# rainerzufalldererste/limg

Measured on AMD Instinct MI355X. Metric: encode Mpixels/s, 8K RGBA (limg_encode3d_test-equivalent: all 11 planes stored), higher is better.
Workload: dtype u8/i32 integer stage + f32 float stage (bit-exact vs the reference's strict SSE build)

## Files before the change

limg_amd/csrc/limg_hip_blocked.hip:

```cpp
#include "limg_hip_device.h"

namespace limg_hip
{
  namespace
  {
    __device__ __forceinline__ void scratch_fence()
    {
      __builtin_amdgcn_fence(__ATOMIC_RELEASE, "workgroup");
      __builtin_amdgcn_fence(__ATOMIC_ACQUIRE, "workgroup");
    }

    struct MState { float nA[4], nB[4], nC[4], invA, invB, invC; };

    template <int CH>
    __device__ __forceinline__ float dot_seq(const float *a, const float *b)
    {
      float sum = 0.0f;
#pragma unroll
      for (int i = 0; i < CH; i++) sum += a[i] * b[i];
      return sum;
    }

    template <int CH>
    __device__ __forceinline__ void m_init(const limg_hip_block_record &r, MState &s)
    {
      bool nzA = false, nzB = false, nzC = false;
#pragma unroll
      for (int i = 0; i < 4; i++) { s.nA[i] = 0.0f; s.nB[i] = 0.0f; s.nC[i] = 0.0f; }
#pragma unroll
      for (int i = 0; i < CH; i++)
      {
        s.nA[i] = (float)((int)r.dirA_max[i] - (int)r.dirA_min[i]);
        s.nB[i] = (float)((int)r.dirB_mag[i] - (int)r.dirB_offset[i]);
        s.nC[i] = (float)((int)r.dirC_mag[i] - (int)r.dirC_offset[i]);
        nzA |= s.nA[i] != 0; nzB |= s.nB[i] != 0; nzC |= s.nC[i] != 0;
      }
      s.invA = nzA ? 1.0f / dot_seq<CH>(s.nA, s.nA) : 0.0f;
      s.invB = nzB ? 1.0f / dot_seq<CH>(s.nB, s.nB) : 0.0f;
      s.invC = nzC ? 1.0f / dot_seq<CH>(s.nC, s.nC) : 0.0f;
    }

    template <int CH>
    __device__ __forceinline__ void m_factors(const float *color, const limg_hip_block_record &in, const MState &s, float f[3])
    {
      float t[4], est[4];
#pragma unroll
      for (int i = 0; i < CH; i++) t[i] = color[i] - (float)in.dirA_min[i];
      f[0] = dot_seq<CH>(t, s.nA) * s.invA;
#pragma unroll
      for (int i = 0; i < CH; i++) { est[i] = (float)in.dirA_min[i] + f[0] * s.nA[i]; t[i] = (color[i] - est[i]) - (float)in.dirB_offset[i]; }
      f[1] = dot_seq<CH>(t, s.nB) * s.invB;
#pragma unroll
      for (int i = 0; i < CH; i++) { est[i] = est[i] + f[1] * s.nB[i]; t[i] = (color[i] - est[i]) - (float)in.dirC_offset[i]; }
      f[2] = dot_seq<CH>(t, s.nC) * s.invC;
    }

    template <typename T>
    __device__ __forceinline__ float2_t splat2(T v) { return float2_t{ (float)v, (float)v }; }
    __device__ __forceinline__ float2_t pair2(float x, float y) { return float2_t{ x, y }; }

    template <int CH, typename TA, typename TB>
    __device__ __forceinline__ float2_t dot_seq2(const TA *a, const TB *b)
    {
      float2_t sum = { 0.0f, 0.0f };
#pragma unroll
      for (int i = 0; i < CH; i++) sum += a[i] * b[i];
      return sum;
    }

    template <int CH, typename TC, typename TR>
    __device__ __forceinline__ void m_factors2(const TC *color, const TR *mnA, const TR *ofB, const TR *ofC, const TR *nA, const TR *nB, const TR *nC, TR invA, TR invB, TR invC,
                                               float2_t f[3])
    {
      float2_t t[4], est[4];
#pragma unroll
      for (int i = 0; i < CH; i++) t[i] = color[i] - mnA[i];
      f[0] = dot_seq2<CH>(t, nA) * invA;
#pragma unroll
      for (int i = 0; i < CH; i++) { est[i] = mnA[i] + f[0] * nA[i]; t[i] = (color[i] - est[i]) - ofB[i]; }
      f[1] = dot_seq2<CH>(t, nB) * invB;
#pragma unroll
      for (int i = 0; i < CH; i++) { est[i] = est[i] + f[1] * nB[i]; t[i] = (color[i] - est[i]) - ofC[i]; }
      f[2] = dot_seq2<CH>(t, nC) * invC;
    }

    template <int CH>
    __device__ void m_matches_pair(const limg_hip_block_record &a, const limg_hip_block_record &b0, const limg_hip_block_record &b1, bool &r0, bool &r1)
    {
      MState sa;
      m_init<CH>(a, sa);
      float amnA[4], aofB[4], aofC[4];
      float2_t nA[4], nB[4], nC[4], mnA[4], ofB[4], ofC[4], avgB[4];
#pragma unroll
      for (int i = 0; i < CH; i++)
      {
        amnA[i] = (float)a.dirA_min[i]; aofB[i] = (float)a.dirB_offset[i]; aofC[i] = (float)a.dirC_offset[i];
        nA[i] = pair2((float)((int)b0.dirA_max[i] - (int)b0.dirA_min[i]), (float)((int)b1.dirA_max[i] - (int)b1.dirA_min[i]));
        nB[i] = pair2((float)((int)b0.dirB_mag[i] - (int)b0.dirB_offset[i]), (float)((int)b1.dirB_mag[i] - (int)b1.dirB_offset[i]));
        nC[i] = pair2((float)((int)b0.dirC_mag[i] - (int)b0.dirC_offset[i]), (float)((int)b1.dirC_mag[i] - (int)b1.dirC_offset[i]));
        mnA[i] = pair2((float)b0.dirA_min[i], (float)b1.dirA_min[i]);
        ofB[i] = pair2((float)b0.dirB_offset[i], (float)b1.dirB_offset[i]);
        ofC[i] = pair2((float)b0.dirC_offset[i], (float)b1.dirC_offset[i]);
        avgB[i] = pair2(b0.avg[i], b1.avg[i]);
      }
      float2_t invBA = 1.0f / dot_seq2<CH>(nA, nA), invBB = 1.0f / dot_seq2<CH>(nB, nB), invBC = 1.0f / dot_seq2<CH>(nC, nC);
      {
        bool zA0 = true, zA1 = true, zB0 = true, zB1 = true, zC0 = true, zC1 = true;
#pragma unroll
        for (int i = 0; i < CH; i++)
        {
          zA0 &= nA[i].x == 0.0f; zA1 &= nA[i].y == 0.0f; zB0 &= nB[i].x == 0.0f; zB1 &= nB[i].y == 0.0f; zC0 &= nC[i].x == 0.0f; zC1 &= nC[i].y == 0.0f;
        }
        invBA = pair2(zA0 ? 0.0f : invBA.x, zA1 ? 0.0f : invBA.y);
        invBB = pair2(zB0 ? 0.0f : invBB.x, zB1 ? 0.0f : invBB.y);
        invBC = pair2(zC0 ? 0.0f : invBC.x, zC1 ? 0.0f : invBC.y);
      }
      const float w[4] = { 2, 4, 3, 3 };
      float lenA[3] = { 3, 3, 3 };
      float2_t avgDiffSq = { 0, 0 }, lenB[3] = { { 3, 3 }, { 3, 3 }, { 3, 3 } };
#pragma unroll
      for (int i = 0; i < CH; i++)
      {
        const float2_t d = a.avg[i] - avgB[i];
        avgDiffSq += d * d * w[i];
        lenA[0] += (sa.nA[i] * sa.nA[i]) * w[i]; lenB[0] += (nA[i] * nA[i]) * w[i];
        lenA[1] += (sa.nB[i] * sa.nB[i]) * w[i]; lenB[1] += (nB[i] * nB[i]) * w[i];
        lenA[2] += (sa.nC[i] * sa.nC[i]) * w[i]; lenB[2] += (nC[i] * nC[i]) * w[i];
      }
      const float sumA = lenA[0] + lenA[1] + lenA[2];
      const float2_t sumB = lenB[0] + lenB[1] + lenB[2];
      const float2_t ratio = (sumA + 1) / (sumB + 1);
      const float maxAvg = (float)(16 * 3 * CH), maxRange = (float)(200 * 3 * CH);
      const bool q0 = avgDiffSq.x < maxAvg && sumA < maxRange && sumB.x < maxRange, q1 = avgDiffSq.y < maxAvg && sumA < maxRange && sumB.y < maxRange;
      const bool j0 = ratio.x > 1.375f || ratio.x < (1.f / 1.375f), j1 = ratio.y > 1.375f || ratio.y < (1.f / 1.375f);
      r0 = q0; r1 = q1;
      if ((q0 || j0) && (q1 || j1)) return;
      float invA[3];
      float2_t invB[3];
#pragma unroll
      for (int i = 0; i < 3; i++) { invA[i] = 1.0f / lenA[i]; invB[i] = 1.0f / lenB[i]; }
#pragma unroll
      for (int i = 1; i < 3; i++) { invA[i] *= 2.f; invB[i] *= 2.f; }
      float2_t fb[3];
      m_factors2<CH>(a.avg, mnA, ofB, ofC, nA, nB, nC, invBA, invBB, invBC, fb);
      const float2_t termB = __builtin_elementwise_abs(fb[0]) * invB[0] + __builtin_elementwise_abs(0.5f - fb[1]) * invB[1] + __builtin_elementwise_abs(0.5f - fb[2]) * invB[2];
      float2_t sum = { 0, 0 };
#pragma unroll 1
      for (int z = 0; z < 3; z++)
#pragma unroll 1
        for (int y = 0; y < 3; y++)
#pragma unroll
          for (int x = 0; x < 3; x++)
          {
            const float xf = x * 0.5f, yf = y * 0.5f, zf = z * 0.5f;
            float2_t color[4], fa[3];
#pragma unroll
            for (int i = 0; i < CH; i++) color[i] = nA[i] * xf + nB[i] * yf + nC[i] * zf;
            m_factors2<CH>(color, amnA, aofB, aofC, sa.nA, sa.nB, sa.nC, sa.invA, sa.invB, sa.invC, fa);
            sum += __builtin_elementwise_abs(fa[0]) * invA[0] + __builtin_elementwise_abs(0.5f - fa[1]) * invA[1] + __builtin_elementwise_abs(0.5f - fa[2]) * invA[2];
            sum += termB;
          }
      const float2_t avgF = sum * (1.f / 27);
      if (!q0 && !j0) r0 = avgF.x < 3.0f;
      if (!q1 && !j1) r1 = avgF.y < 3.0f;
    }

    template <int CH>
    __device__ __forceinline__ int m_early(const limg_hip_block_record &a, const MState &sa, const limg_hip_block_record &b)
    {
      MState sb;
      m_init<CH>(b, sb);
      const float w[4] = { 2, 4, 3, 3 };
      float avgDiffSq = 0, lenA[3] = { 3, 3, 3 }, lenB[3] = { 3, 3, 3 };
#pragma unroll
      for (int i = 0; i < CH; i++)
      {
        const float d = a.avg[i] - b.avg[i];
        avgDiffSq += d * d * w[i];
        lenA[0] += (sa.nA[i] * sa.nA[i]) * w[i]; lenB[0] += (sb.nA[i] * sb.nA[i]) * w[i];
        lenA[1] += (sa.nB[i] * sa.nB[i]) * w[i]; lenB[1] += (sb.nB[i] * sb.nB[i]) * w[i];
        lenA[2] += (sa.nC[i] * sa.nC[i]) * w[i]; lenB[2] += (sb.nC[i] * sb.nC[i]) * w[i];
      }
      const float sumA = lenA[0] + lenA[1] + lenA[2], sumB = lenB[0] + lenB[1] + lenB[2];
      const float ratio = (sumA + 1) / (sumB + 1);
      const float maxAvg = (float)(16 * 3 * CH), maxRange = (float)(200 * 3 * CH);
      if (avgDiffSq < maxAvg && sumA < maxRange && sumB < maxRange) return 1;
      if (ratio > 1.375f || ratio < (1.f / 1.375f)) return 2;
      return 0;
    }

    __device__ __forceinline__ void cell_to_block(const BlockedParams &p, uint32_t sx, uint32_t sy, int cell, bool &ok, size_t &idx)
    {
      const int dy = cell / kMatchSide - kMatchLo, dx = cell - (cell / kMatchSide) * kMatchSide - kMatchLo;
      const uint32_t cx = sx + (uint32_t)dx, cy = sy + (uint32_t)dy;
      ok = cell < kMatchCells && (dx | dy) != 0 && cx < p.blocksX && cy < p.blocksY;
      idx = ok ? (size_t)cy * p.blocksX + cx : 0;
    }

    template <int CH>
    __global__ __launch_bounds__(256) void k_blocked_bounds(const BlockedParams p)
    {
      const uint32_t i = blockIdx.x * 256 + threadIdx.x;
      if (i >= p.blocksX * p.blocksY) return;
      const limg_hip_block_record r = p.pass1[i];
      MState s;
      m_init<CH>(r, s);
      const float w[4] = { 2, 4, 3, 3 };
      float len[3] = { 3, 3, 3 }, qA = 0, qB = 0, qC = 0, qM = 0, qOB = 0, qOC = 0;
#pragma unroll
      for (int k = 0; k < CH; k++)
      {
        len[0] += (s.nA[k] * s.nA[k]) * w[k]; len[1] += (s.nB[k] * s.nB[k]) * w[k]; len[2] += (s.nC[k] * s.nC[k]) * w[k];
        qA += s.nA[k] * s.nA[k]; qB += s.nB[k] * s.nB[k]; qC += s.nC[k] * s.nC[k];
        const float m = (float)r.dirA_min[k], ob = (float)r.dirB_offset[k], oc = (float)r.dirC_offset[k];
        qM += m * m; qOB += ob * ob; qOC += oc * oc;
      }
      const float NA = sqrtf(qA), NB = sqrtf(qB), NC = sqrtf(qC), OB = sqrtf(qOB), OC = sqrtf(qOC);
      float alpha = 0.5f * 2.0f / len[1] + 0.5f * 2.0f / len[2], beta = 0;
      if (qA > 0) beta += 1.0f / (NA * len[0]);
      if (qB > 0) { alpha += (OB / NB) * 2.0f / len[1]; beta += 4.0f / (NB * len[1]); }
      if (qC > 0) { alpha += ((OB + OC) / NC) * 2.0f / len[2]; beta += 8.0f / (NC * len[2]); }
      reinterpret_cast<float4 *>(p.matchBound)[i] = make_float4(alpha, beta, sqrtf(qM), (NA + NB + NC) * 1.0001f);
    }

    template <int CH>
    __global__ __launch_bounds__(256, 3) void k_blocked_match(const BlockedParams p)
    {
      __shared__ unsigned short sList[4][kMatchWords * 64];
      __shared__ unsigned long long sWords[4][kMatchWords];
      const int wave = threadIdx.x >> 6;
      const uint32_t seed = p.seedBase + blockIdx.x * 4 + wave;
      const int lane = lane_id();
      if (seed >= p.seedBase + p.seedCount) return;
      const uint32_t sy = seed / p.blocksX, sx = seed - sy * p.blocksX;
      const limg_hip_block_record a = p.pass1[seed];
      MState sa;
      m_init<CH>(a, sa);
      float boundA = 0, boundB = 0, boundM = 0, boundAvg = 0, boundT0 = 0;
      if (p.matchBound)
      {
        const float4 ba = reinterpret_cast<const float4 *>(p.matchBound)[seed];
        float q = 0;
#pragma unroll
        for (int k = 0; k < CH; k++) q += a.avg[k] * a.avg[k];
        boundA = ba.x; boundB = ba.y; boundM = ba.z; boundAvg = sqrtf(q);
        const float w[4] = { 2, 4, 3, 3 }, zero[4] = { 0, 0, 0, 0 };
        float len[3] = { 3, 3, 3 }, f0[3];
#pragma unroll
        for (int k = 0; k < CH; k++) { len[0] += (sa.nA[k] * sa.nA[k]) * w[k]; len[1] += (sa.nB[k] * sa.nB[k]) * w[k]; len[2] += (sa.nC[k] * sa.nC[k]) * w[k]; }
        m_factors<CH>(zero, a, sa, f0);
        boundT0 = fabsf(f0[0]) * (1.0f / len[0]) + fabsf(0.5f - f0[1]) * ((1.0f / len[1]) * 2.f) + fabsf(0.5f - f0[2]) * ((1.0f / len[2]) * 2.f);
      }
      uint32_t count = 0;
      for (int c = 0; c < kMatchWords; c++)
      {
        const int cell = c * 64 + lane;
        bool ok;
        size_t idx;
        cell_to_block(p, sx, sy, cell, ok, idx);
        int e = 2;
        if (ok) e = m_early<CH>(a, sa, p.pass1[idx]);
        if (e == 0 && p.matchBound)
        {
          const float4 bb = reinterpret_cast<const float4 *>(p.matchBound)[idx];
          const float UA = boundA + boundB * (bb.w + boundM), U = UA + (bb.x + bb.y * (boundAvg + bb.z));
          if (U * 1.01f < 2.5f) e = 1;
          else if (boundT0 - 1.01f * (0.5f * boundB * bb.w) - 0.01f * UA > 3.01f) e = 2;
        }
        const unsigned long long yes = __builtin_amdgcn_ballot_w64(e == 1), open = __builtin_amdgcn_ballot_w64(e == 0);
        if (lane == 0) sWords[wave][c] = yes;
        if (e == 0) sList[wave][count + __builtin_amdgcn_mbcnt_hi((uint32_t)(open >> 32), __builtin_amdgcn_mbcnt_lo((uint32_t)open, 0u))] = (unsigned short)cell;
        count += (uint32_t)__builtin_popcountll(open);
      }
      wave_lds_fence();
      for (uint32_t k = 0; k < count; k += 128)
      {
        const uint32_t i0 = k + lane, i1 = k + 64 + lane;
        const bool v0 = i0 < count, v1 = i1 < count;
        const int cell0 = sList[wave][v0 ? i0 : 0], cell1 = sList[wave][v1 ? i1 : 0];
        bool ok0, ok1, r0 = false, r1 = false;
        size_t idx0, idx1;
        cell_to_block(p, sx, sy, cell0, ok0, idx0);
        cell_to_block(p, sx, sy, cell1, ok1, idx1);
        m_matches_pair<CH>(a, p.pass1[idx0], p.pass1[idx1], r0, r1);
        if (v0 && r0) atomicOr(&sWords[wave][cell0 >> 6], 1ull << (cell0 & 63));
        if (v1 && r1) atomicOr(&sWords[wave][cell1 >> 6], 1ull << (cell1 & 63));
      }
      wave_lds_fence();
      if (lane < kMatchWords) p.matchBits[(size_t)seed * kMatchWords + lane] = sWords[wave][lane];
      if (lane == 0)
      {
        auto bit = [&](int dx, int dy) -> uint32_t { const int cell = (dy + kMatchLo) * kMatchSide + dx + kMatchLo; return (uint32_t)(sWords[wave][cell >> 6] >> (cell & 63)) & 1u; };
        const uint32_t all8 = bit(1, 0) & bit(2, 0) & bit(0, 1) & bit(1, 1) & bit(2, 1) & bit(0, 2) & bit(1, 2) & bit(2, 2);
        p.matchFlags[seed] = (uint8_t)(all8 | ((bit(1, 0) | bit(0, 1)) << 1));
      }
    }

    struct Geo { uint32_t px0, py0, xpx, ypx, n; };

    __device__ __forceinline__ Geo region_geo(const BlockedParams &p, const RegionDesc &R)
    {
      Geo g;
      g.px0 = R.ox * kBlock; g.py0 = R.oy * kBlock;
      g.xpx = R.rx * kBlock; g.ypx = R.ry * kBlock;
      if (R.ox + R.rx == p.blocksX && (p.sizeX % kBlock)) g.xpx = g.xpx - kBlock + p.sizeX % kBlock;
      if (R.oy + R.ry == p.blocksY && (p.sizeY % kBlock)) g.ypx = g.ypx - kBlock + p.sizeY % kBlock;
      g.n = g.xpx * g.ypx;
      return g;
    }

    __device__ __forceinline__ float bcast(float v, int l) { return __int_as_float(__builtin_amdgcn_readlane(__float_as_int(v), l)); }

    __device__ __forceinline__ uint64_t wave_sum64(uint64_t v)
    {
      const uint32_t lo = (uint32_t)v, hi = (uint32_t)(v >> 32);
      return (uint64_t)wave_sum(lo & 0xFFFFu) + ((uint64_t)wave_sum(lo >> 16) << 16) + ((uint64_t)wave_sum(hi) << 32);
    }

    template <int CH>
    __global__ __launch_bounds__(64) void k_blocked_fit_search(const BlockedParams p)
    {
      __shared__ __attribute__((aligned(16))) float s_park[4][64 + 4];
      const uint32_t r = p.order ? p.order[blockIdx.x] : blockIdx.x;
      const int lane = lane_id();
      const RegionDesc R = p.regions[r];
      const Geo g = region_geo(p, R);
      const uint32_t n = g.n, cap = p.scratchCap;
      uint32_t *spx = p.scratchPx + R.scratch;
      uint8_t *sf = p.scratchFac + R.scratch;
      const unsigned short *tab = d_rsqrt_x86_tab;

      uint32_t s0 = 0, s1 = 0, s2 = 0, s3 = 0;
      for (uint32_t i = lane; i < n; i += 64)
      {
        const uint32_t row = i / g.xpx, col = i - row * g.xpx;
        const uint32_t px = p.in[(size_t)(g.py0 + row) * p.sizeX + g.px0 + col];
        spx[i] = px;
        s0 += px & 0xFF; s1 += (px >> 8) & 0xFF; s2 += (px >> 16) & 0xFF; s3 += px >> 24;
      }
      scratch_fence();

      limg_hip_block_record rec;
      memset(&rec, 0, sizeof(rec));
      if (R.keep)
      {
        rec = p.pass1[(size_t)R.oy * p.blocksX + R.ox];
      }
      else
      {
        s0 = wave_sum(s0); s1 = wave_sum(s1); s2 = wave_sum(s2); s3 = wave_sum(s3);
        const float inv_count = 1.0f / (float)n;
        V4 avg;
        avg.a = float2_t{ (float)(int)s0, (float)(int)s2 } * inv_count;
        avg.b = float2_t{ (float)(int)s1, CH == 4 ? (float)(int)s3 : 0.0f } * inv_count;
        const V4 zero4 = { float2_t{ 0.0f, 0.0f }, float2_t{ 0.0f, 0.0f } };
        V4 dirA = zero4, dirB = zero4, dirC = zero4;
        float mm[6] = { 0, 0, 0, 0, 0, 0 };
        bool zeroA = true, zeroB = true, zeroC = true;

        float walk = 0.0f;
        auto park_and_walk = [&](const V4 &u, uint32_t count ) {
          s_park[0][lane] = u.a.x; s_park[1][lane] = u.a.y; s_park[2][lane] = u.b.x; s_park[3][lane] = u.b.y;
          wave_lds_fence();
          if (lane < 4)
          {
            const float *src = s_park[lane];
            if (count == 64u)
            {
#pragma unroll
              for (int h = 0; h < 4; h++)
              {
                float4 v[4];
#pragma unroll
                for (int q = 0; q < 4; q++) v[q] = *reinterpret_cast<const float4 *>(src + 16 * h + 4 * q);
#pragma unroll
                for (int q = 0; q < 4; q++) { walk = walk + v[q].x; walk = walk + v[q].y; walk = walk + v[q].z; walk = walk + v[q].w; }
              }
            }
            else
              for (uint32_t i = 0; i < count; i++) walk = walk + src[i];
          }
          wave_lds_fence();
        };
        auto serial_sum = [&]() -> V4 {
          const float s = walk * inv_count;
          walk = 0.0f;
          V4 d;
          d.a = float2_t{ bcast(s, 0), bcast(s, 1) };
          d.b = float2_t{ bcast(s, 2), bcast(s, 3) };
          return d;
        };
        auto is_zero = [](const V4 &d) { return d.a.x == 0.0f && d.a.y == 0.0f && d.b.x == 0.0f && d.b.y == 0.0f; };

        for (uint32_t base = 0; base < n; base += 64)
        {
          const uint32_t i = base + lane;
          const bool active = i < n;
          const V4 pf = px_to_v4(active ? spx[i] : 0u);
          V4 d = pf - avg;
          mask_alpha<CH>(d);
          const V4 u = unit4<CH>(tab, d, active);
          park_and_walk(u, min(64u, n - base));
        }
        dirA = serial_sum();
        zeroA = is_zero(dirA);
        if (!zeroA)
        {
          const float invA = 1.0f / dp4<CH>(dirA, dirA);
          float mn = 0.0f, mx = 0.0f;
          for (uint32_t base = 0; base < n; base += 64)
          {
            const uint32_t i = base + lane;
            const bool active = i < n;
            const V4 pf = px_to_v4(active ? spx[i] : 0u);
            const float fA = dp4<CH>(pf - avg, dirA) * invA;
            if (active) { mn = vmin(mn, fA); mx = vmax(mx, fA); }
            V4 e = pf - (avg + dirA * fA);
            mask_alpha<CH>(e);
            const V4 u = unit4<CH>(tab, e, active);
            park_and_walk(u, min(64u, n - base));
          }
          wave_min_max(mn, mx);
          mm[0] = mn; mm[1] = mx;
          dirB = serial_sum();
          zeroB = is_zero(dirB);
          if (!zeroB)
          {
            const float invB = 1.0f / dp4<CH>(dirB, dirB);
            float mnB = FLT_MAX, mxB = -FLT_MAX, mnC = FLT_MAX, mxC = -FLT_MAX;
            if (CH == 4)
            {
              V4 est0 = zero4;
              for (uint32_t base = 0; base < n; base += 64)
              {
                const uint32_t i = base + lane;
                const bool active = i < n;
                const V4 pf = px_to_v4(active ? spx[i] : 0u);
                const float fA = dp4<CH>(pf - avg, dirA) * invA;
                const V4 est = avg + dirA * fA;
                const float fB = dp4<CH>(pf - est, dirB) * invB;
                if (active) { mnB = vmin(mnB, fB); mxB = vmax(mxB, fB); }
                const V4 est2 = est + dirB * fB;
                const V4 u = unit4<CH>(tab, pf - est2, active);
                park_and_walk(u, min(64u, n - base));
                if (base == 0) est0 = est2;
              }
              wave_min_max(mnB, mxB);
              est0.a = float2_t{ bcast(est0.a.x, 0), bcast(est0.a.y, 0) };
              est0.b = float2_t{ bcast(est0.b.x, 0), bcast(est0.b.y, 0) };
              dirC = serial_sum();
              zeroC = is_zero(dirC);
              if (!zeroC)
              {
                const float invC = 1.0f / dp4<CH>(dirC, dirC);
                for (uint32_t base = 0; base < n; base += 64)
                {
                  const uint32_t i = base + lane;
                  const bool active = i < n;
                  const V4 pf = px_to_v4(active ? spx[i] : 0u);
                  const float fC = dp4<CH>(pf - est0, dirC) * invC;
                  if (active) { mnC = vmin(mnC, fC); mxC = vmax(mxC, fC); }
                }
                wave_min_max(mnC, mxC);
              }
            }
            else
            {
              dirC.a.x = dirA.b.x * dirB.a.y - dirA.a.y * dirB.b.x;
              dirC.b.x = dirA.a.y * dirB.a.x - dirA.a.x * dirB.a.y;
              dirC.a.y = dirA.a.x * dirB.b.x - dirA.b.x * dirB.a.x;
              dirC.b.y = 0.0f;
              zeroC = dirC.a.x == 0.0f && dirC.b.x == 0.0f && dirC.a.y == 0.0f;
              const float invC = zeroC ? 0.0f : 1.0f / dp4<CH>(dirC, dirC);
              for (uint32_t base = 0; base < n; base += 64)
              {
                const uint32_t i = base + lane;
                const bool active = i < n;
                const V4 pf = px_to_v4(active ? spx[i] : 0u);
                const float fA = dp4<CH>(pf - avg, dirA) * invA;
                const V4 est = avg + dirA * fA;
                const float fB = dp4<CH>(pf - est, dirB) * invB;
                if (active) { mnB = vmin(mnB, fB); mxB = vmax(mxB, fB); }
                if (!zeroC)
                {
                  const V4 e = pf - (est + dirB * fB);
                  const float fC = dp4<CH>(e, dirC) * invC;
                  if (active) { mnC = vmin(mnC, fC); mxC = vmax(mxC, fC); }
                }
              }
              wave_min_max(mnB, mxB);
              if (!zeroC) wave_min_max(mnC, mxC);
            }
            mm[2] = mnB; mm[3] = mxB;
            if (!zeroC) { mm[4] = mnC; mm[5] = mxC; }
          }
        }
        const float av[4] = { avg.a.x, avg.b.x, avg.a.y, avg.b.y };
        const float dA[4] = { dirA.a.x, dirA.b.x, dirA.a.y, dirA.b.y }, dB[4] = { dirB.a.x, dirB.b.x, dirB.a.y, dirB.b.y }, dC[4] = { dirC.a.x, dirC.b.x, dirC.a.y, dirC.b.y };
        const bool deadA = zeroA, deadB = zeroA || zeroB, deadC = deadB || zeroC;
#pragma unroll
        for (int c = 0; c < 4; c++)
        {
          rec.avg[c] = (CH == 3 && c == 3) ? 0.0f : av[c];
          if (CH == 3 && c == 3) continue;
          rec.dirA_min[c] = (int16_t)cvt_rne(av[c] + (deadA ? 0.0f : mm[0] * dA[c]));
          rec.dirA_max[c] = (int16_t)cvt_rne(av[c] + (deadA ? 0.0f : mm[1] * dA[c]));
          rec.dirB_offset[c] = (int16_t)cvt_rne(deadB ? 0.0f : mm[2] * dB[c]);
          rec.dirB_mag[c] = (int16_t)cvt_rne(deadB ? 0.0f : mm[3] * dB[c]);
          rec.dirC_offset[c] = (int16_t)cvt_rne(deadC ? 0.0f : mm[4] * dC[c]);
          rec.dirC_mag[c] = (int16_t)cvt_rne(deadC ? 0.0f : mm[5] * dC[c]);
        }
      }

      const int16_t *lo3[3] = { rec.dirA_min, rec.dirB_offset, rec.dirC_offset }, *hi3[3] = { rec.dirA_max, rec.dirB_mag, rec.dirC_mag };
      V4 nrm[3], off[3];
      float invN[3];
      RecU ru;
#pragma unroll
      for (int f = 0; f < 3; f++)
      {
        float nv[4], ov[4];
#pragma unroll
        for (int c = 0; c < 4; c++) { nv[c] = (float)((int)hi3[f][c] - (int)lo3[f][c]); ov[c] = (float)lo3[f][c]; }
        float s = ((0.0f + nv[0] * nv[0]) + nv[1] * nv[1]) + nv[2] * nv[2];
        if (CH == 4) s = s + nv[3] * nv[3];
        const bool nz = nv[0] != 0.0f || nv[1] != 0.0f || nv[2] != 0.0f || (CH == 4 && nv[3] != 0.0f);
        invN[f] = nz ? 1.0f / s : 0.0f;
        nrm[f].a = float2_t{ nv[0], nv[2] }; nrm[f].b = float2_t{ nv[1], nv[3] };
        off[f].a = float2_t{ ov[0], ov[2] }; off[f].b = float2_t{ ov[1], ov[3] };
      }
#pragma unroll
      for (int c = 0; c < 3; c++)
      {
        ru.nA[c] = (int)rec.dirA_max[c] - (int)rec.dirA_min[c]; ru.nB[c] = (int)rec.dirB_mag[c] - (int)rec.dirB_offset[c]; ru.nC[c] = (int)rec.dirC_mag[c] - (int)rec.dirC_offset[c];
        ru.mA[c] = (int)(((uint32_t)(int)rec.dirA_min[c] << 8) + 128u); ru.mB[c] = (int)(((uint32_t)(int)rec.dirB_offset[c] << 8) + 128u);
        ru.mC[c] = (int)(((uint32_t)(int)rec.dirC_offset[c] << 8) + 128u);
      }

      for (uint32_t base = 0; base < n; base += 64)
      {
        const uint32_t i = base + lane;
        if (i >= n) continue;
        const V4 pv = px_to_v4(spx[i]);
        const float fa = dp4<CH>(pv - off[0], nrm[0]) * invN[0];
        V4 est = off[0] + nrm[0] * fa;
        const float fb = dp4<CH>((pv - est) - off[1], nrm[1]) * invN[1];
        est = est + nrm[1] * fb;
        const float fc = dp4<CH>((pv - est) - off[2], nrm[2]) * invN[2];
        sf[i] = (uint8_t)cvt_u8_rne_sat(255.0f * fa);
        sf[(size_t)cap + i] = (uint8_t)cvt_u8_rne_sat(255.0f * fb);
        sf[2 * (size_t)cap + i] = (uint8_t)cvt_u8_rne_sat(255.0f * fc);
      }
      scratch_fence();

      uint32_t shift[3] = { 0, 0, 0 };
      if (p.forced[0] >= 0)
      {
        shift[0] = (uint32_t)p.forced[0]; shift[1] = (uint32_t)p.forced[1]; shift[2] = (uint32_t)p.forced[2];
      }
      else if (p.crushBits)
      {
        const uint64_t maxBlockN = p.maxBlock * (uint64_t)n;
        auto T = [&](uint32_t a, uint32_t b, uint32_t c, uint64_t &be) -> bool {
          uint64_t acc = 0;
          for (uint32_t base = 0; base < n; base += 64)
          {
            const uint32_t i = base + lane;
            uint32_t err = 0;
            if (i < n) err = trial_error(spx[i], sf[i], sf[(size_t)cap + i], sf[2 * (size_t)cap + i], ru, a, b, c);
            if (__builtin_amdgcn_ballot_w64(err > p.maxPixel32) != 0ull) return false;
            acc += err;
          }
          be = wave_sum64(acc);
          return be * 16ull < maxBlockN;
        };
        if (p.fast) search_fast<uint64_t>(T, shift);
        else search_accurate<uint64_t>(T, shift);
      }
      const uint32_t calls = (shift[0] && shift[0] != 8 ? 1u : 0u) + (shift[1] && shift[1] != 8 ? 1u : 0u) + (shift[2] && shift[2] != 8 ? 1u : 0u);
      if (lane == 0)
      {
        RegionOut o;
        o.rec = rec;
        o.shiftWord = shift[0] | (shift[1] << 8) | (shift[2] << 16) | (calls << 24);
        o.pad[0] = o.pad[1] = o.pad[2] = 0;
        p.out[r] = o;
      }
    }

    __global__ __launch_bounds__(1024) void k_blocked_order(const BlockedParams p)
    {
      __shared__ uint32_t sBins[1024], sWaveSmall[16];
      __shared__ uint32_t sLarge, sCarry;
      const int tid = threadIdx.x, lane = lane_id(), wave = tid >> 6;
      const uint32_t n = p.nRegions;
      sBins[tid] = 0;
      if (tid == 0) sCarry = 0;
      __syncthreads();
      for (uint32_t i = tid; i < n; i += 1024)
      {
        const uint32_t nb = p.regions[i].rx * p.regions[i].ry;
        if (nb > 4u) atomicAdd(&sBins[nb < 1023u ? nb : 1023u], 1u);
      }
      __syncthreads();
      uint32_t own = sBins[tid], suf = own;
      for (int off = 1; off < 1024; off <<= 1)
      {
        __syncthreads();
        sBins[tid] = suf;
        __syncthreads();
        if (tid + off < 1024) suf += sBins[tid + off];
      }
      __syncthreads();
      sBins[tid] = suf - own;
      if (tid == 0) sLarge = suf;
      __syncthreads();
      const uint32_t nLarge = sLarge;
      for (uint32_t base = 0; base < n; base += 1024)
      {
        const uint32_t i = base + tid;
        uint32_t nb = 0;
        if (i < n) nb = p.regions[i].rx * p.regions[i].ry;
        const bool small = i < n && nb <= 4u;
        if (i < n && !small) p.order[atomicAdd(&sBins[nb < 1023u ? nb : 1023u], 1u)] = i;
        const uint64_t m = __builtin_amdgcn_ballot_w64(small);
        if (lane == 0) sWaveSmall[wave] = (uint32_t)__builtin_popcountll(m);
        __syncthreads();
        uint32_t before = sCarry;
        for (int w = 0; w < wave; w++) before += sWaveSmall[w];
        if (small) p.order[nLarge + before + (uint32_t)__builtin_popcountll(m & ((1ull << lane) - 1ull))] = i;
        __syncthreads();
        if (tid == 0)
        {
          uint32_t t = sCarry;
          for (int w = 0; w < 16; w++) t += sWaveSmall[w];
          sCarry = t;
        }
        __syncthreads();
      }
    }

    template <int CH>
    __global__ __launch_bounds__(64) void k_blocked_store(const BlockedParams p)
    {
      const uint32_t r = p.order ? p.order[blockIdx.x] : blockIdx.x;
      const int lane = lane_id();
      const RegionDesc R = p.regions[r];
      const Geo g = region_geo(p, R);
      const uint32_t n = g.n, cap = p.scratchCap;
      const uint8_t *sf = p.scratchFac + R.scratch;
      const RegionOut O = p.out[r];
      const limg_hip_block_record &rec = O.rec;
      const uint32_t shift[3] = { O.shiftWord & 0xFF, (O.shiftWord >> 8) & 0xFF, (O.shiftWord >> 16) & 0xFF };

      const int16_t *vec[6] = { rec.dirA_min, rec.dirA_max, rec.dirB_offset, rec.dirB_mag, rec.dirC_offset, rec.dirC_mag };
      uint32_t col[6];
#pragma unroll
      for (int k = 0; k < 6; k++)
      {
        uint32_t v = 0;
#pragma unroll
        for (int c = 0; c < CH; c++)
        {
          int q = (int)vec[k][c] + (k >= 2 ? 0x80 : 0);
          q = q < 0 ? 0 : (q > 255 ? 255 : q);
          v |= (uint32_t)q << (8 * c);
        }
        if (CH == 3) v |= 0xFF000000u;
        col[k] = v;
      }
      const uint32_t pa = shift[0] == 8 ? 0xFFu : shift[0] * 0x22u, pb = shift[1] == 8 ? 0xFFu : shift[1] * 0x22u, pc = shift[2] == 8 ? 0xFFu : shift[2] * 0x22u;
      const uint32_t shiftVal = 0xFF000000u | (pa << 16) | (pb << 8) | pc;
      const uint64_t bits = (uint64_t)(CH * 18 + CH * 8 + 32) + (uint64_t)n * ((8 - shift[0]) + (8 - shift[1]) + (8 - shift[2]));
      const uint8_t bpp = (uint8_t)((bits + n / 2) / n);
      const uint32_t blockIndex = 0xFF000000u | (p.regionBase + r + 1u);
      int nn[3][4], mc[3][4];
#pragma unroll
      for (int f = 0; f < 3; f++)
#pragma unroll
        for (int c = 0; c < 4; c++)
        {
          int nv = (int)vec[2 * f + 1][c] - (int)vec[2 * f][c], m = (int)vec[2 * f][c];
          if (c < 3) { if (shift[f] > 7) { nv = 0; if (f > 0) m = 0; } }
          else if (CH == 3) { nv = 0; m = 0xFFFF; }
          nn[f][c] = nv;
          mc[f][c] = (int)(((uint32_t)m << 8) + 128u);
        }
      const int mulA = (int)shift_mul(shift[0]), mulB = (int)shift_mul(shift[1]), mulC = (int)shift_mul(shift[2]);
      const uint8_t *nz[3];
      {
        const uint8_t *q = p.noise + p.noiseBase[r];
#pragma unroll
        for (int k = 0; k < 3; k++)
        {
          nz[k] = q;
          if (shift[k] != 0 && shift[k] != 8) q += n;
        }
      }

      if (p.vecStore)
      {
        for (uint32_t base = 0; base < n; base += 256)
        {
          const uint32_t i = base + (uint32_t)lane * 4u;
          if (i >= n) continue;
          const uint32_t row = i / g.xpx, colx = i - row * g.xpx;
          const size_t o = (size_t)(g.py0 + row) * p.sizeX + g.px0 + colx;
          uint32_t fq[3];
#pragma unroll
          for (int k = 0; k < 3; k++)
          {
            uint32_t f4 = *reinterpret_cast<const uint32_t *>(sf + (size_t)k * cap + i);
            const uint32_t s = shift[k];
            if (s != 0 && s != 8)
            {
              const uint32_t z4 = *reinterpret_cast<const uint32_t *>(nz[k] + i);
              uint32_t out = 0;
#pragma unroll
              for (int q = 0; q < 4; q++)
              {
                int t = (int)((f4 >> (8 * q)) & 0xFFu) + ((int)((z4 >> (8 * q)) & ((1u << s) - 1u)) - (int)(1u << (s - 1)));
                t = t < 0 ? 0 : (t > 255 ? 255 : t);
                out |= ((uint32_t)t >> s) << (8 * q);
              }
              f4 = out;
            }
            fq[k] = f4;
          }
          uint32_t st[3];
#pragma unroll
          for (int k = 0; k < 3; k++) st[k] = shift[k] > 7 ? 0u : ((fq[k] << shift[k]) & ((0xFFu << shift[k]) & 0xFFu) * 0x01010101u);
          *reinterpret_cast<uint32_t *>(p.info.pFactorsA + o) = st[0];
          *reinterpret_cast<uint32_t *>(p.info.pFactorsB + o) = st[1];
          *reinterpret_cast<uint32_t *>(p.info.pFactorsC + o) = st[2];
          *reinterpret_cast<uint32_t *>(p.info.pBitsPerPixel + o) = (uint32_t)bpp * 0x01010101u;
          *reinterpret_cast<uint4 *>(p.info.pShiftABCX + o) = make_uint4(shiftVal, shiftVal, shiftVal, shiftVal);
          *reinterpret_cast<uint4 *>(p.info.pColAMin + o) = make_uint4(col[0], col[0], col[0], col[0]);
          *reinterpret_cast<uint4 *>(p.info.pColAMax + o) = make_uint4(col[1], col[1], col[1], col[1]);
          *reinterpret_cast<uint4 *>(p.info.pColBMin + o) = make_uint4(col[2], col[2], col[2], col[2]);
          *reinterpret_cast<uint4 *>(p.info.pColBMax + o) = make_uint4(col[3], col[3], col[3], col[3]);
          *reinterpret_cast<uint4 *>(p.info.pColCMin + o) = make_uint4(col[4], col[4], col[4], col[4]);
          *reinterpret_cast<uint4 *>(p.info.pColCMax + o) = make_uint4(col[5], col[5], col[5], col[5]);
          *reinterpret_cast<uint4 *>(p.info.pBlockIndex + o) = make_uint4(blockIndex, blockIndex, blockIndex, blockIndex);
          uint32_t dec[4];
#pragma unroll
          for (int q = 0; q < 4; q++)
          {
            const int dA = (int)((fq[0] >> (8 * q)) & 0xFFu) * mulA, dB = (int)((fq[1] >> (8 * q)) & 0xFFu) * mulB, dC = (int)((fq[2] >> (8 * q)) & 0xFFu) * mulC;
            uint32_t decoded = 0;
#pragma unroll
            for (int c = 0; c < 4; c++)
            {
              int est = (mad_i24(dA, nn[0][c], mc[0][c]) >> 8) + (mad_i24(dB, nn[1][c], mc[1][c]) >> 8) + (mad_i24(dC, nn[2][c], mc[2][c]) >> 8);
              est = est < 0 ? 0 : (est > 255 ? 255 : est);
              decoded |= (uint32_t)est << (8 * c);
            }
            dec[q] = decoded;
          }
          *reinterpret_cast<uint4 *>(p.info.pDecoded + o) = make_uint4(dec[0], dec[1], dec[2], dec[3]);
        }
        return;
      }
      for (uint32_t base = 0; base < n; base += 64)
      {
        const uint32_t i = base + lane;
        if (i >= n) continue;
        const uint32_t row = i / g.xpx, colx = i - row * g.xpx;
        const size_t o = (size_t)(g.py0 + row) * p.sizeX + g.px0 + colx;
        uint32_t v[3];
#pragma unroll
        for (int k = 0; k < 3; k++)
        {
          uint32_t f = sf[(size_t)k * cap + i];
          const uint32_t s = shift[k];
          if (s != 0 && s != 8)
          {
            int t = (int)f + ((int)(nz[k][i] & ((1u << s) - 1u)) - (int)(1u << (s - 1)));
            t = t < 0 ? 0 : (t > 255 ? 255 : t);
            f = (uint32_t)t >> s;
          }
          v[k] = f;
        }
        p.info.pFactorsA[o] = (uint8_t)(v[0] << shift[0]);
        p.info.pFactorsB[o] = (uint8_t)(v[1] << shift[1]);
        p.info.pFactorsC[o] = (uint8_t)(v[2] << shift[2]);
        p.info.pBitsPerPixel[o] = bpp;
        p.info.pShiftABCX[o] = shiftVal;
        p.info.pColAMin[o] = col[0]; p.info.pColAMax[o] = col[1]; p.info.pColBMin[o] = col[2];
        p.info.pColBMax[o] = col[3]; p.info.pColCMin[o] = col[4]; p.info.pColCMax[o] = col[5];
        p.info.pBlockIndex[o] = blockIndex;
        const int dA = (int)v[0] * mulA, dB = (int)v[1] * mulB, dC = (int)v[2] * mulC;
        uint32_t decoded = 0;
#pragma unroll
        for (int c = 0; c < 4; c++)
        {
          int est = (mad_i24(dA, nn[0][c], mc[0][c]) >> 8) + (mad_i24(dB, nn[1][c], mc[1][c]) >> 8) + (mad_i24(dC, nn[2][c], mc[2][c]) >> 8);
          est = est < 0 ? 0 : (est > 255 ? 255 : est);
          decoded |= (uint32_t)est << (8 * c);
        }
        p.info.pDecoded[o] = decoded;
      }
    }
  }

  void launch_blocked_bounds(const BlockedParams &p, hipStream_t s)
  {
    const uint32_t blocks = p.blocksX * p.blocksY;
    if (blocks == 0 || !p.matchBound) return;
    if (p.channels == 4) hipLaunchKernelGGL(k_blocked_bounds<4>, dim3((blocks + 255) / 256), dim3(256), 0, s, p);
    else hipLaunchKernelGGL(k_blocked_bounds<3>, dim3((blocks + 255) / 256), dim3(256), 0, s, p);
  }

  void launch_blocked_match(const BlockedParams &p, hipStream_t s)
  {
    if (p.seedCount == 0) return;
    const dim3 grid((p.seedCount + 3) / 4), block(256);
    if (p.channels == 4) hipLaunchKernelGGL(k_blocked_match<4>, grid, block, 0, s, p);
    else hipLaunchKernelGGL(k_blocked_match<3>, grid, block, 0, s, p);
  }

  void launch_blocked_fit_search(const BlockedParams &p, hipStream_t s)
  {
    if (p.nRegions == 0) return;
    if (p.channels == 4) hipLaunchKernelGGL(k_blocked_fit_search<4>, dim3(p.nRegions), dim3(64), 0, s, p);
    else hipLaunchKernelGGL(k_blocked_fit_search<3>, dim3(p.nRegions), dim3(64), 0, s, p);
  }

  void launch_blocked_order(const BlockedParams &p, hipStream_t s)
  {
    if (p.nRegions == 0 || !p.order) return;
    hipLaunchKernelGGL(k_blocked_order, dim3(1), dim3(1024), 0, s, p);
  }

  void launch_blocked_store(const BlockedParams &p, hipStream_t s)
  {
    if (p.nRegions == 0) return;
    if (p.channels == 4) hipLaunchKernelGGL(k_blocked_store<4>, dim3(p.nRegions), dim3(64), 0, s, p);
    else hipLaunchKernelGGL(k_blocked_store<3>, dim3(p.nRegions), dim3(64), 0, s, p);
  }
}
```

limg_amd/csrc/limg_hip_blocked_api.hip:

```cpp
#include "limg_hip_context.h"

#include <chrono>
#include <condition_variable>
#include <functional>

using namespace limg_hip;

namespace
{
  using clk = std::chrono::steady_clock;
  double ms(clk::time_point a, clk::time_point b) { return std::chrono::duration<double, std::milli>(b - a).count(); }
  bool add_elapsed(double &ms, hipEvent_t a, hipEvent_t b) { float t = 0; if (hipEventElapsedTime(&t, a, b) != hipSuccess) return false; ms += t; return true; }

  constexpr size_t kInFlight = 32;
  constexpr uint32_t kBands = 16;

  template <class F> void for_each_written_plane(F &&f)
  {
    using I = limg_hip_blocked_encode3d_info;
    auto each = [&](auto... m) { (f(m), ...); };
    each(&I::pDecoded, &I::pFactorsA, &I::pFactorsB, &I::pFactorsC, &I::pBitsPerPixel, &I::pShiftABCX, &I::pColAMin, &I::pColAMax, &I::pColBMin, &I::pColBMax, &I::pColCMin,
         &I::pColCMax, &I::pBlockIndex);
  }
  bool has_written_planes(const limg_hip_blocked_encode3d_info &info) { bool all = true; for_each_written_plane([&](auto m) { all = all && info.*m; }); return all; }

  size_t copy_regions(const std::vector<HostRegion> &regs, limg_hip_region *pRegions, size_t capacity)
  {
    for (size_t i = 0; pRegions && i < regs.size() && i < capacity; i++) pRegions[i] = { regs[i].ox, regs[i].oy, regs[i].rx, regs[i].ry };
    return regs.size();
  }

  struct BlockedJob
  {
    limg_hip_context *c;
    hipStream_t s;
    size_t sizeX, sizeY, blocks, maxCalls;
    uint32_t blocksX, blocksY, bandRows, nBands;
    int channels; bool pcg;
    bool compact;
    BlockedParams bp;
    hipEvent_t *frontTimers;
    limg_hip_block_record *hRec; unsigned long long *hBits; uint8_t *hFlags;
    RegionDesc *desc; RegionOut *hOut; unsigned long long *noiseBase;
    unsigned long long *callState, *callOff, *dCallState, *dCallOff;
    uint32_t *callPx, *dCallPx;
    uint32_t *npx;
  };

  limg_hip_result set_up(BlockedJob &j, limg_hip_context *c, const uint32_t *pIn, size_t sizeX, size_t sizeY, int hasAlpha, const limg_hip_blocked_encode3d_info &info,
                         uint32_t errorFactor, int fastBitCrushing, void *stream, bool compact)
  {
    j.compact = compact;
    j.c = c; j.s = (hipStream_t)stream; j.sizeX = sizeX; j.sizeY = sizeY; j.channels = hasAlpha ? 4 : 3; j.pcg = c->opt.dither_pcg != 0;
    j.blocksX = (uint32_t)((sizeX + kBlock - 1) / kBlock); j.blocksY = (uint32_t)((sizeY + kBlock - 1) / kBlock);
    j.blocks = (size_t)j.blocksX * j.blocksY; j.maxCalls = 3 * j.blocks;
    j.bandRows = (j.blocksY + kBands - 1) / kBands; j.nBands = (j.blocksY + j.bandRows - 1) / j.bandRows;
    const uint64_t capMax = ((uint64_t)sizeX * sizeY + 3ull * j.blocks + 3ull) & ~3ull;
    if (capMax > 0xFFFFFFF0ull) return limg_hip_error_InvalidParameter;
    BlockedParams &bp = j.bp;
    memset(&bp, 0, sizeof(bp));
    bp.in = pIn; bp.sizeX = (uint32_t)sizeX; bp.sizeY = (uint32_t)sizeY; bp.blocksX = j.blocksX; bp.blocksY = j.blocksY; bp.channels = (uint32_t)j.channels;
    const uint64_t maxPixel = (uint64_t)0x6 * (errorFactor / 2) * 7, maxBlock = (uint64_t)0x4 * (errorFactor / 2) * 7;
    bp.maxPixel32 = maxPixel > 0xFFFFFFFFull ? 0xFFFFFFFFu : (uint32_t)maxPixel;
    bp.maxBlock = maxBlock;
    bp.crushBits = errorFactor != 0; bp.fast = fastBitCrushing != 0;
    const bool forced = c->opt.forced_shift[0] >= 0 && c->opt.forced_shift[0] <= 8 && c->opt.forced_shift[1] >= 0 && c->opt.forced_shift[1] <= 8 &&
                        c->opt.forced_shift[2] >= 0 && c->opt.forced_shift[2] <= 8;
    for (int i = 0; i < 3; i++) bp.forced[i] = forced ? c->opt.forced_shift[i] : -1;
    bp.info = info;
    bp.scratchCap = (uint32_t)capMax;
    uintptr_t w = 0, b8 = 0;
    for_each_written_plane([&](auto m) { (sizeof(*(info.*m)) == 4 ? w : b8) |= (uintptr_t)(info.*m); });
    bp.vecStore = (sizeX % kBlock == 0 && sizeY % kBlock == 0 && (w & 15u) == 0 && (b8 & 3u) == 0 && TOPT(c, blocked_no_vec_store) == 0) ? 1 : 0;
    return limg_hip_success;
  }

  limg_hip_result ensure_events(std::vector<hipEvent_t> &events, size_t n, unsigned flags)
  { for (hipEvent_t e; events.size() < n; events.push_back(e)) HIP_TRY(hipEventCreateWithFlags(&e, flags)); return limg_hip_success; }
  limg_hip_result ensure_stream(hipStream_t &stream) { if (!stream) HIP_TRY(hipStreamCreateWithFlags(&stream, hipStreamNonBlocking)); return limg_hip_success; }

  limg_hip_result ensure_resources(BlockedJob &j)
  {
    limg_hip_context *c = j.c;
    const size_t blocks = j.blocks, maxCalls = j.maxCalls, px = j.sizeX * j.sizeY, capMax = j.bp.scratchCap;
    const bool bound = TOPT(c, blocked_no_bound) == 0;
    limg_hip_result r = ensure_events(c->workTimers, 4 * kInFlight + 3, hipEventDefault);
    auto need = [&r](auto &buf, size_t bytes) { if (r == limg_hip_success) r = buf.ensure(bytes); };
    need(c->bMatch, blocks * kMatchWords * 8); need(c->bFlags, blocks); need(c->hFlags, blocks + 16);
    if (bound) need(c->bBound, blocks * 16);
    need(c->hRec, blocks * sizeof(limg_hip_block_record)); need(c->hBits, blocks * kMatchWords * 8);
    if (r == limg_hip_success) r = ensure_events(c->bandEvents, 2 * kBands + 1, hipEventDisableTiming);
    need(c->hDesc, blocks * sizeof(RegionDesc)); need(c->hOut, blocks * sizeof(RegionOut)); need(c->hNoiseBase, blocks * 8 + 8);
    need(c->hNoise, maxCalls * 20 + 64); need(c->bCalls, maxCalls * 20 + 64);
    need(c->bRegions, blocks * sizeof(RegionDesc)); need(c->bOut, blocks * sizeof(RegionOut)); need(c->bNoiseBase, blocks * 8 + 8); need(c->bOrder, blocks * 4);
    need(c->bNoise, 3 * px + 64); need(c->bPx, capMax * 4); need(c->bFac, capMax * 3);
    for (hipStream_t *st : { &c->copyStream, &c->searchStream, &c->storeStream })
      if (r == limg_hip_success) r = ensure_stream(*st);
    if (r == limg_hip_success) r = ensure_events(c->workEvents, kInFlight, hipEventDisableTiming);
    if (r != limg_hip_success) return r;
    try { c->regionPx.resize(blocks); }
    catch (const std::bad_alloc &) { return limg_hip_error_MemoryAllocationFailure; }
    j.npx = c->regionPx.data();
    j.frontTimers = c->workTimers.data() + 4 * kInFlight;
    j.hRec = (limg_hip_block_record *)c->hRec.p; j.hBits = (unsigned long long *)c->hBits.p; j.hFlags = (uint8_t *)c->hFlags.p;
    j.desc = (RegionDesc *)c->hDesc.p; j.hOut = (RegionOut *)c->hOut.p; j.noiseBase = (unsigned long long *)c->hNoiseBase.p;
    j.callState = (unsigned long long *)c->hNoise.p; j.callOff = j.callState + maxCalls; j.callPx = (uint32_t *)(j.callOff + maxCalls);
    j.dCallState = (unsigned long long *)c->bCalls.p; j.dCallOff = j.dCallState + maxCalls; j.dCallPx = (uint32_t *)(j.dCallOff + maxCalls);
    j.bp.matchBits = (unsigned long long *)c->bMatch.p; j.bp.matchFlags = (uint8_t *)c->bFlags.p;
    if (bound) j.bp.matchBound = (float *)c->bBound.p;
    j.bp.scratchPx = (uint32_t *)c->bPx.p; j.bp.scratchFac = (uint8_t *)c->bFac.p; j.bp.noise = (const uint8_t *)c->bNoise.p;
    return limg_hip_success;
  }

  limg_hip_result similarity_bands(BlockedJob &j)
  {
    limg_hip_context *c = j.c;
    BlockedParams &bp = j.bp;
    const hipStream_t s = j.s, cs = c->copyStream;
    HIP_TRY(hipEventRecord(j.frontTimers[1], s));
    c->lastBlocks = j.blocks;
    launch_blocked_bounds(bp, s);
    for (uint32_t b = 0; b < j.nBands; b++)
    {
      const uint32_t row0 = b * j.bandRows, rows = min(j.bandRows, j.blocksY - row0);
      bp.seedBase = row0 * j.blocksX; bp.seedCount = rows * j.blocksX;
      launch_blocked_match(bp, s);
      HIP_TRY(hipGetLastError());
      HIP_TRY(hipEventRecord(c->bandEvents[2 * b], s));
      HIP_TRY(hipStreamWaitEvent(cs, c->bandEvents[2 * b], 0));
      HIP_TRY(hipMemcpyAsync(j.hBits + (size_t)bp.seedBase * kMatchWords, bp.matchBits + (size_t)bp.seedBase * kMatchWords, (size_t)bp.seedCount * kMatchWords * 8,
                             hipMemcpyDeviceToHost, cs));
      HIP_TRY(hipMemcpyAsync(j.hFlags + bp.seedBase, bp.matchFlags + bp.seedBase, bp.seedCount, hipMemcpyDeviceToHost, cs));
      HIP_TRY(hipEventRecord(c->bandEvents[2 * b + 1], cs));
      if (b == 1 || (b == 0 && j.nBands == 1))
      {
        HIP_TRY(hipMemcpyAsync(j.hRec, c->records.p, j.blocks * sizeof(limg_hip_block_record), hipMemcpyDeviceToHost, cs));
        HIP_TRY(hipEventRecord(c->bandEvents[2 * kBands], cs));
      }
    }
    HIP_TRY(hipEventRecord(j.frontTimers[2], s));
    HIP_TRY(hipEventSynchronize(c->bandEvents[1]));
    return limg_hip_success;
  }

  struct Pipe { std::mutex m; std::condition_variable cv; size_t ready = 0; bool finished = false; };

  struct Merge
  {
    BlockedJob &j;
    Pipe &pipe;
    uint32_t bandsReady = 0;
    bool recordsHere = false, bandError = false, failed = false;
    size_t laid = 0; uint64_t cap = 0;
    clk::time_point end;
    void need_records() { if (!recordsHere && hipEventSynchronize(j.c->bandEvents[2 * kBands]) != hipSuccess) bandError = true; recordsHere = true; }
    void need_seed_row(uint32_t row)
    {
      for (; bandsReady < j.nBands && row >= bandsReady * j.bandRows; bandsReady++)
        if (hipEventSynchronize(j.c->bandEvents[2 * bandsReady + 1]) != hipSuccess) bandError = true;
    }
    void publish(size_t count)
    {
      for (size_t i = laid; i < count; i++)
      {
        const HostRegion &h = j.c->lastRegions[i];
        size_t xpx = (size_t)h.rx * kBlock, ypx = (size_t)h.ry * kBlock;
        if (h.ox + h.rx == j.blocksX && (j.sizeX % kBlock)) xpx = xpx - kBlock + j.sizeX % kBlock;
        if (h.oy + h.ry == j.blocksY && (j.sizeY % kBlock)) ypx = ypx - kBlock + j.sizeY % kBlock;
        j.npx[i] = (uint32_t)(xpx * ypx);
        j.desc[i] = { h.ox, h.oy, h.rx, h.ry, h.keep, (uint32_t)cap, { 0, 0 } };
        cap += ((uint64_t)j.npx[i] + 3) & ~3ull;
      }
      laid = count;
      { std::lock_guard<std::mutex> lk(pipe.m); pipe.ready = count; }
      pipe.cv.notify_one();
    }
    void run() noexcept
    {
      try
      {
        const std::function<void()> records = [this] { need_records(); };
        const std::function<void(uint32_t)> seedRow = [this](uint32_t row) { need_seed_row(row); };
        const std::function<void(size_t)> progress = [this](size_t count) { publish(count); };
        blocked_merge(j.hRec, j.hBits, j.blocksX, j.blocksY, j.channels, j.c->lastRegions, &progress, &seedRow, j.hFlags, &records);
      }
      catch (...) { failed = true; }
      need_seed_row(j.blocksY - 1);
      need_records();
      end = clk::now();
      { std::lock_guard<std::mutex> lk(pipe.m); pipe.finished = true; }
      pipe.cv.notify_one();
    }
  };

  struct Worker
  {
    struct Batch { size_t r0, r1, ev; };
    const BlockedJob &j;
    Pipe &pipe;
    limg_hip_context *const c = j.c;
    Batch queue[kInFlight];
    size_t head = 0, tail = 0, issued = 0;
    bool fin = false;
    uint64_t chain = kDitherSeed, noiseOff = 0; size_t callCount = 0;
    double kernelMs[2] = { 0, 0 };
    double busy[3] = { 0, 0, 0 };
    bool storeTimed[kInFlight] = {};
    limg_hip_result result = limg_hip_success;
    static constexpr size_t kOrderFrom = 512;
    static constexpr size_t kWorthWithOneInFlight = 16384, kWorthFromInsideAWalk = 8192, kWalkPiece = 2048;
    BlockedParams params_of(const Batch &b) const
    {
      BlockedParams q = j.bp;
      q.regions = (const RegionDesc *)c->bRegions.p + b.r0; q.nRegions = (uint32_t)(b.r1 - b.r0); q.regionBase = (uint32_t)b.r0;
      q.out = (RegionOut *)c->bOut.p + b.r0; q.noiseBase = (const unsigned long long *)c->bNoiseBase.p + b.r0;
      q.order = (b.r1 - b.r0 >= kOrderFrom && TOPT(c, blocked_no_order) == 0) ? (uint32_t *)c->bOrder.p + b.r0 : nullptr;
      return q;
    }
    void enqueue_published(bool mayWait, size_t minNew)
    {
      if (fin || tail - head >= kInFlight) return;
      size_t r0 = 0, r1 = 0;
      {
        std::unique_lock<std::mutex> lk(pipe.m);
        if (mayWait) pipe.cv.wait(lk, [&] { return pipe.ready > issued || pipe.finished; });
        if (pipe.ready == issued) fin = pipe.finished;
        else if (pipe.ready - issued >= minNew || pipe.finished) { r0 = issued; r1 = issued = pipe.ready; }
      }
      if (r1 == r0) return;
      const Batch nb = { r0, r1, tail % kInFlight };
      if (storeTimed[nb.ev])
        if (hipEventSynchronize(c->workTimers[4 * nb.ev + 3]) == hipSuccess) add_elapsed(kernelMs[1], c->workTimers[4 * nb.ev + 2], c->workTimers[4 * nb.ev + 3]);
      storeTimed[nb.ev] = false;
      if (result == limg_hip_success)
      {
        const size_t n = r1 - r0;
        const BlockedParams q = params_of(nb);
        const hipStream_t bs = c->searchStream;
        bool ok = hipMemcpyAsync((RegionDesc *)c->bRegions.p + r0, j.desc + r0, n * sizeof(RegionDesc), hipMemcpyHostToDevice, bs) == hipSuccess;
        ok = ok && hipEventRecord(c->workTimers[4 * nb.ev], bs) == hipSuccess;
        if (ok) { launch_blocked_order(q, bs); launch_blocked_fit_search(q, bs); ok = hipGetLastError() == hipSuccess; }
        ok = ok && hipEventRecord(c->workTimers[4 * nb.ev + 1], bs) == hipSuccess;
        ok = ok && hipMemcpyAsync(j.hOut + r0, (RegionOut *)c->bOut.p + r0, n * sizeof(RegionOut), hipMemcpyDeviceToHost, bs) == hipSuccess;
        ok = ok && hipEventRecord(c->workEvents[nb.ev], bs) == hipSuccess;
        if (!ok) result = limg_hip_error_Generic;
      }
      queue[tail++ % kInFlight] = nb;
    }
    void walk_and_store(const Batch pending, clk::time_point w0)
    {
      if (result != limg_hip_success) return;
      bool ok = hipEventSynchronize(c->workEvents[pending.ev]) == hipSuccess;
      if (ok) add_elapsed(kernelMs[0], c->workTimers[4 * pending.ev], c->workTimers[4 * pending.ev + 1]);
      const clk::time_point w1 = clk::now();
      const size_t call0 = callCount;
      for (size_t w = pending.r0; ok && w < pending.r1; w += kWalkPiece)
      {
        const size_t n = pending.r1 - w < kWalkPiece ? pending.r1 - w : kWalkPiece;
        chain = chain_walk_batch(chain, n, reinterpret_cast<const uint8_t *>(&j.hOut[w].shiftWord), sizeof(RegionOut), j.npx + w, j.noiseBase + w, j.callState, j.callOff,
                                 j.callPx, noiseOff, callCount, j.maxCalls, j.pcg);
        if (w + n < pending.r1) enqueue_published(false, kWorthFromInsideAWalk);
      }
      const clk::time_point w2 = clk::now();
      const size_t nc = callCount - call0;
      const hipStream_t ss = c->storeStream;
      ok = ok && hipStreamWaitEvent(ss, c->workEvents[pending.ev], 0) == hipSuccess;
      ok = ok && hipEventRecord(c->workTimers[4 * pending.ev + 2], ss) == hipSuccess;
      if (ok && nc)
      {
        ok = hipMemcpyAsync(j.dCallState + call0, j.callState + call0, nc * 8, hipMemcpyHostToDevice, ss) == hipSuccess &&
             hipMemcpyAsync(j.dCallOff + call0, j.callOff + call0, nc * 8, hipMemcpyHostToDevice, ss) == hipSuccess &&
             hipMemcpyAsync(j.dCallPx + call0, j.callPx + call0, nc * 4, hipMemcpyHostToDevice, ss) == hipSuccess;
        if (ok) { launch_noise_expand_calls((uint8_t *)c->bNoise.p, j.dCallState + call0, j.dCallOff + call0, j.dCallPx + call0, nc, j.pcg, ss); ok = hipGetLastError() == hipSuccess; }
      }
      ok = ok && hipMemcpyAsync((unsigned long long *)c->bNoiseBase.p + pending.r0, j.noiseBase + pending.r0, (pending.r1 - pending.r0) * 8, hipMemcpyHostToDevice, ss) == hipSuccess;
      if (ok && !j.compact) { launch_blocked_store(params_of(pending), ss); ok = hipGetLastError() == hipSuccess; }
      if (ok && hipEventRecord(c->workTimers[4 * pending.ev + 3], ss) == hipSuccess) storeTimed[pending.ev] = true;
      const clk::time_point w3 = clk::now();
      busy[0] += ms(w0, w1); busy[1] += ms(w1, w2); busy[2] += ms(w2, w3);
      if (!ok) result = limg_hip_error_Generic;
    }
    void run() noexcept
    {
      if (hipSetDevice(c->device) != hipSuccess) result = limg_hip_error_Generic;
      for (;;)
      {
        const clk::time_point w0 = clk::now();
        enqueue_published(head == tail, head == tail ? 0 : kWorthWithOneInFlight);
        if (head < tail) walk_and_store(queue[head++ % kInFlight], w0);
        if (fin && head == tail) break;
      }
      if (hipStreamSynchronize(c->searchStream) != hipSuccess && result == limg_hip_success) result = limg_hip_error_Generic;
      if (hipStreamSynchronize(c->storeStream) != hipSuccess && result == limg_hip_success) result = limg_hip_error_Generic;
      for (size_t i = 0; i < kInFlight; i++)
        if (storeTimed[i]) add_elapsed(kernelMs[1], c->workTimers[4 * i + 2], c->workTimers[4 * i + 3]);
    }
  };

  void collect_stats(const BlockedJob &j)
  {
    limg_hip_context *c = j.c;
    memset(c->statsHost, 0, sizeof(c->statsHost));
    for (size_t i = 0; i < c->lastRegions.size(); i++)
      for (int f = 0; f < 3; f++)
      {
        uint32_t sh = (j.hOut[i].shiftWord >> (8 * f)) & 0xFFu;
        if (sh > 8) sh = 8;
        c->statsHost[f] += (uint64_t)(8 - sh) * j.npx[i];
        c->statsHost[3 + 9 * f + sh] += j.npx[i];
      }
    c->statsState = 2; c->statsPixels = (uint64_t)j.sizeX * j.sizeY;
  }
}

extern "C"
{
  int limg_hip_host_blocked_matches(int channels, const limg_hip_block_record *pSeed, const limg_hip_block_record *pCandidate)
  {
    if (!pSeed || !pCandidate || (channels != 3 && channels != 4)) return -1;
    return blocked_matches_host(channels, *pSeed, *pCandidate) ? 1 : 0;
  }

  limg_hip_result limg_hip_host_blocked_merge(const limg_hip_block_record *pFits, const uint64_t *pMatchBits, size_t blocksX, size_t blocksY, int channels, limg_hip_region *pRegions,
                                              size_t capacity, size_t *pCount)
  {
    if (!pFits || !pCount) return limg_hip_error_ArgumentNull;
    if (blocksX == 0 || blocksY == 0 || blocksX > 0x0FFFFFFFull || blocksY > 0x0FFFFFFFull || (channels != 3 && channels != 4)) return limg_hip_error_InvalidParameter;
    std::vector<HostRegion> regs;
    std::vector<uint8_t> flags;
    if (pMatchBits)
    {
      flags.resize(blocksX * blocksY + 16);
      for (size_t i = 0; i < blocksX * blocksY; i++)
      {
        const uint64_t *w = pMatchBits + i * kMatchWords;
        auto bit = [&](int dx, int dy) -> unsigned { const int cell = (dy + kMatchLo) * kMatchSide + dx + kMatchLo; return (unsigned)(w[cell >> 6] >> (cell & 63)) & 1u; };
        const unsigned all8 = bit(1, 0) & bit(2, 0) & bit(0, 1) & bit(1, 1) & bit(2, 1) & bit(0, 2) & bit(1, 2) & bit(2, 2);
        flags[i] = (uint8_t)(all8 | ((bit(1, 0) | bit(0, 1)) << 1));
      }
    }
    blocked_merge(pFits, (const unsigned long long *)pMatchBits, (uint32_t)blocksX, (uint32_t)blocksY, channels, regs, nullptr, nullptr, pMatchBits ? flags.data() : nullptr);
    *pCount = copy_regions(regs, pRegions, capacity);
    return limg_hip_success;
  }

  size_t limg_hip_host_blocked_match_words(void) { return kMatchWords; }

  limg_hip_result limg_hip_host_blocked_match_bits(const limg_hip_block_record *pFits, size_t blocksX, size_t blocksY, int channels, uint64_t *pMatchBits)
  {
    if (!pFits || !pMatchBits) return limg_hip_error_ArgumentNull;
    if (channels != 3 && channels != 4) return limg_hip_error_InvalidParameter;
    for (size_t sy = 0; sy < blocksY; sy++)
      for (size_t sx = 0; sx < blocksX; sx++)
      {
        uint64_t *w = pMatchBits + (sy * blocksX + sx) * kMatchWords;
        for (int i = 0; i < kMatchWords; i++) w[i] = 0;
        for (int cell = 0; cell < kMatchCells; cell++)
        {
          const long dy = cell / kMatchSide - kMatchLo, dx = cell % kMatchSide - kMatchLo;
          const long cx = (long)sx + dx, cy = (long)sy + dy;
          if ((dx | dy) == 0 || cx < 0 || cy < 0 || cx >= (long)blocksX || cy >= (long)blocksY) continue;
          if (blocked_matches_host(channels, pFits[sy * blocksX + sx], pFits[(size_t)cy * blocksX + cx])) w[cell >> 6] |= 1ull << (cell & 63);
        }
      }
    return limg_hip_success;
  }

  limg_hip_result limg_hip_blocked_encode3d_device(limg_hip_context *c, const uint32_t *pIn, size_t sizeX, size_t sizeY, int hasAlpha, const limg_hip_blocked_encode3d_info *pInfo,
                                                   uint32_t errorFactor, int fastBitCrushing, void *stream)
  {
    if (!c || !pIn || !pInfo || !has_written_planes(*pInfo)) return limg_hip_error_ArgumentNull;
    return blocked_encode_device(c, pIn, sizeX, sizeY, hasAlpha, pInfo, errorFactor, fastBitCrushing, (hipStream_t)stream);
  }
}

namespace limg_hip
{
  limg_hip_result blocked_encode_device(limg_hip_context *c, const uint32_t *pIn, size_t sizeX, size_t sizeY, int hasAlpha, const limg_hip_blocked_encode3d_info *pInfo,
                                        uint32_t errorFactor, int fastBitCrushing, hipStream_t stream)
  {
    const limg_hip_blocked_encode3d_info noPlanes = {};
    if (sizeX == 0 || sizeY == 0 || sizeX > 0x7FFFFFF8ull || sizeY > 0x7FFFFFF8ull || sizeX * sizeY > 0x60000000ull) return limg_hip_error_InvalidParameter;
    HIP_TRY(hipSetDevice(c->device));
    const clk::time_point t0 = clk::now();
    BlockedJob j; limg_hip_result r;
    if ((r = set_up(j, c, pIn, sizeX, sizeY, hasAlpha, pInfo ? *pInfo : noPlanes, errorFactor, fastBitCrushing, stream, pInfo == nullptr)) != limg_hip_success) return r;
    if ((r = ensure_resources(j)) != limg_hip_success) return r;
    c->blockedScratchCap = j.bp.scratchCap; c->packTimed = false; c->lastBlocked.valid = false;
    EncodeExtra x1; x1.fitOnly = true;
    HIP_TRY(hipEventRecord(j.frontTimers[0], j.s));
    if ((r = encode_device(c, pIn, sizeX, sizeY, hasAlpha, nullptr, nullptr, errorFactor, 0, fastBitCrushing, j.s, x1)) != limg_hip_success) return r;
    j.bp.pass1 = (const limg_hip_block_record *)c->records.p;
    if ((r = similarity_bands(j)) != limg_hip_success) { (void)hipStreamSynchronize(c->copyStream); return r; }
    const clk::time_point t1 = clk::now();
    Pipe pipe;
    Merge merge{ j, pipe };
    Worker worker{ j, pipe };
    run_on_threads(2, [&](unsigned t) { if (t == 0) merge.run(); else worker.run(); });
    const clk::time_point t5 = clk::now();
    double a = 0, b = 0;
    const bool ok = add_elapsed(a, j.frontTimers[0], j.frontTimers[1]) && add_elapsed(b, j.frontTimers[1], j.frontTimers[2]);
    c->blockedKernelMs[0] = ok ? a : 0; c->blockedKernelMs[1] = ok ? b : 0; c->blockedKernelMs[2] = worker.kernelMs[0]; c->blockedKernelMs[3] = worker.kernelMs[1];
    c->blockedMs[0] = ms(t0, t1); c->blockedMs[1] = ms(t1, merge.end); c->blockedMs[2] = worker.busy[0]; c->blockedMs[3] = worker.busy[1]; c->blockedMs[4] = worker.busy[2];
    c->blockedMs[5] = ms(t0, t5);
    if (merge.failed) return limg_hip_error_MemoryAllocationFailure;
    if (merge.bandError) return limg_hip_error_Generic;
    if (worker.result == limg_hip_success && c->opt.collect_stats) collect_stats(j);
    c->lastBlocked.sizeX = sizeX; c->lastBlocked.sizeY = sizeY; c->lastBlocked.channels = j.channels; c->lastBlocked.errorFactor = errorFactor;
    c->lastBlocked.flags = (fastBitCrushing ? 1u : 0u) | (j.pcg ? 2u : 0u);
    c->lastBlocked.valid = worker.result == limg_hip_success;
    return worker.result;
  }
}

extern "C"
{

  limg_hip_result limg_hip_blocked_regions(limg_hip_context *c, limg_hip_region *pRegions, size_t capacity, size_t *pCount)
  {
    if (!c || !pCount) return limg_hip_error_ArgumentNull;
    *pCount = copy_regions(c->lastRegions, pRegions, capacity);
    return limg_hip_success;
  }

  limg_hip_result limg_hip_blocked_timing(limg_hip_context *c, double *pMs6)
  {
    if (!c || !pMs6) return limg_hip_error_ArgumentNull;
    memcpy(pMs6, c->blockedMs, sizeof(c->blockedMs));
    return limg_hip_success;
  }

  limg_hip_result limg_hip_blocked_match_bits(limg_hip_context *c, uint64_t *pBits, size_t capacityWords, size_t *pWords)
  {
    if (!c || !pWords) return limg_hip_error_ArgumentNull;
    std::lock_guard<std::recursive_mutex> hostLock(c->hostEntry);
    const size_t words = c->lastBlocks * kMatchWords;
    *pWords = words;
    if (pBits && c->hBits.p) memcpy(pBits, c->hBits.p, (words < capacityWords ? words : capacityWords) * 8);
    return limg_hip_success;
  }

  limg_hip_result limg_hip_blocked_kernel_timing(limg_hip_context *c, double *pMs4)
  {
    if (!c || !pMs4) return limg_hip_error_ArgumentNull;
    if (c->packTimed)
    {
      float t = 0;
      if (hipEventSynchronize(c->packTimers[1]) == hipSuccess && hipEventElapsedTime(&t, c->packTimers[0], c->packTimers[1]) == hipSuccess) c->blockedKernelMs[3] += t;
      c->packTimed = false;
    }
    memcpy(pMs4, c->blockedKernelMs, sizeof(c->blockedKernelMs));
    return limg_hip_success;
  }

  limg_hip_result limg_hip_blocked_encode3d_stats(limg_hip_context *c, const uint32_t *pIn, size_t sizeX, size_t sizeY, int hasAlpha, limg_hip_blocked_encode3d_info *pInfo,
                                                  uint32_t errorFactor, int fastBitCrushing, uint64_t *pCounters30, uint64_t *pPixels)
  {
    if (!c || !pCounters30) return limg_hip_error_ArgumentNull;
    std::lock_guard<std::recursive_mutex> hostLock(c->hostEntry);
    const int32_t was = c->opt.collect_stats;
    c->opt.collect_stats = 1;
    limg_hip_result r = limg_hip_blocked_encode3d(c, pIn, sizeX, sizeY, hasAlpha, pInfo, errorFactor, fastBitCrushing);
    if (r == limg_hip_success) r = limg_hip_last_stats(c, pCounters30, pPixels);
    c->opt.collect_stats = was;
    return r;
  }

  limg_hip_result limg_hip_blocked_encode3d(limg_hip_context *c, const uint32_t *pIn, size_t sizeX, size_t sizeY, int hasAlpha, limg_hip_blocked_encode3d_info *pInfo, uint32_t errorFactor,
                                            int fastBitCrushing)
  {
    if (!c || !pIn || !pInfo) return limg_hip_error_ArgumentNull;
    std::lock_guard<std::recursive_mutex> hostLock(c->hostEntry);
    if (sizeX == 0 || sizeY == 0) return limg_hip_error_InvalidParameter;
    HIP_TRY(hipSetDevice(c->device));
    const size_t px = sizeX * sizeY, stride = (px * 4 + 255) & ~(size_t)255;
    limg_hip_result r;
    if ((r = c->in.ensure(px * 4)) != limg_hip_success) return r;
    if ((r = c->planes.ensure(stride * 13)) != limg_hip_success) return r;
    HIP_TRY(hipMemcpy(c->in.p, pIn, px * 4, hipMemcpyHostToDevice));
    if (!has_written_planes(*pInfo)) return limg_hip_error_ArgumentNull;
    limg_hip_blocked_encode3d_info d = {};
    size_t i = 0;
    for_each_written_plane([&](auto m) { d.*m = (std::decay_t<decltype(d.*m)>)((uint8_t *)c->planes.p + stride * i++); });
    if ((r = limg_hip_blocked_encode3d_device(c, (const uint32_t *)c->in.p, sizeX, sizeY, hasAlpha, &d, errorFactor, fastBitCrushing, nullptr)) != limg_hip_success) return r;
    if ((r = limg_hip_check_device_status(c)) != limg_hip_success) return r;
    hipError_t e = hipSuccess;
    for_each_written_plane([&](auto m) { if (e == hipSuccess) e = hipMemcpy(pInfo->*m, d.*m, px * sizeof(*(d.*m)), hipMemcpyDeviceToHost); });
    HIP_TRY(e);
    return limg_hip_success;
  }
}
```

limg_amd/csrc/limg_hip_blocked_host.h:

```cpp
#ifndef LIMG_HIP_BLOCKED_HOST_H
#define LIMG_HIP_BLOCKED_HOST_H

#include <stddef.h>
#include <stdint.h>

#include <functional>
#include <vector>

#include "../../include/limg_hip.h"

namespace limg_hip
{
  constexpr int kMatchLo = 5, kMatchHi = 12;
  constexpr int kMatchSide = kMatchLo + kMatchHi + 1;
  constexpr int kMatchCells = kMatchSide * kMatchSide;
  constexpr int kMatchWords = (kMatchCells + 63) / 64;

  struct HostRegion { uint32_t ox, oy, rx, ry, keep; };

  void blocked_merge(const limg_hip_block_record *pass1, const unsigned long long *matchBits, uint32_t blocksX, uint32_t blocksY, int channels, std::vector<HostRegion> &out,
                     const std::function<void(size_t)> *progress = nullptr, const std::function<void(uint32_t)> *needSeedRow = nullptr, const uint8_t *seedFlags = nullptr,
                     const std::function<void()> *needRecords = nullptr);
  bool blocked_matches_host(int channels, const limg_hip_block_record &seed, const limg_hip_block_record &cand);
  uint64_t chain_walk_batch(uint64_t h, size_t count, const uint8_t *shiftWords, size_t stride, const uint32_t *npx, unsigned long long *noiseBase, unsigned long long *callState,
                            unsigned long long *callOff, uint32_t *callPx, uint64_t &noiseOff, size_t &callCount, size_t maxCalls, bool pcg);
}

#endif
```

limg_amd/csrc/limg_hip_context.h:

```cpp
#ifndef LIMG_HIP_CONTEXT_H
#define LIMG_HIP_CONTEXT_H

#include "limg_hip_internal.h"
#ifdef LIMG_HIP_TEST_HOOKS
#include "../../include/limg_hip_test_hooks.h"
#define TOPT(c, member) ((c)->topt.member)
#else
#define TOPT(c, member) 0
#endif
#include "limg_hip_rccl.h"

#include <stddef.h>
#include <stdio.h>
#include <string.h>
#include <new>
#include <mutex>
#include <thread>
#include <vector>

#define HIP_TRY(expr)                                                                                                     \
  do                                                                                                                      \
  {                                                                                                                       \
    const hipError_t e_ = (expr);                                                                                         \
    if (e_ != hipSuccess)                                                                                                 \
    {                                                                                                                     \
      fprintf(stderr, "limg_hip: %s failed: %s (%s:%d)\n", #expr, hipGetErrorString(e_), __FILE__, __LINE__);            \
      return limg_hip_error_Generic;                                                                                      \
    }                                                                                                                     \
  } while (0)

struct DevBuf
{
  void *p = nullptr;
  size_t cap = 0;
  limg_hip_result ensure(size_t bytes)
  {
    if (bytes <= cap) return limg_hip_success;
    if (p) (void)hipFree(p);
    p = nullptr; cap = 0;
    if (hipMalloc(&p, bytes) != hipSuccess) { p = nullptr; return limg_hip_error_MemoryAllocationFailure; }
    cap = bytes;
    return limg_hip_success;
  }
  void release() { if (p) (void)hipFree(p); p = nullptr; cap = 0; }
};

struct HostBuf
{
  void *p = nullptr;
  size_t cap = 0;
  limg_hip_result ensure(size_t bytes)
  {
    if (bytes <= cap) return limg_hip_success;
    if (p) (void)hipHostFree(p);
    p = nullptr; cap = 0;
    const size_t want = bytes + bytes / 4;
    if (hipHostMalloc(&p, want, hipHostMallocDefault) != hipSuccess) { p = nullptr; return limg_hip_error_MemoryAllocationFailure; }
    cap = want;
    return limg_hip_success;
  }
  void release() { if (p) (void)hipHostFree(p); p = nullptr; cap = 0; }
};

struct limg_hip_context
{
  std::recursive_mutex hostEntry;
  int device = 0;
  limg_hip_options opt;
#ifdef LIMG_HIP_TEST_HOOKS
  limg_hip_test_options topt;
#endif
  DevBuf records, shifts, stripCalls, stripBase;
  DevBuf invN;
  DevBuf noise;
  bool noisePcg = false;
  size_t noiseCount = 0;
  uint64_t noiseNext = limg_hip::kDitherSeed;
  DevBuf noiseDyn;
  DevBuf noiseStates;
  DevBuf noiseCk;
  size_t noiseCkCount = 0;
  std::vector<uint64_t> noiseCkHost;
  DevBuf park;
  DevBuf batchTable;
  hipStream_t fitStream = nullptr;
  std::vector<hipEvent_t> pipeEvents;
  HostBuf hStage;
  hipEvent_t hStageEvent = nullptr;
  bool hStageBusy = false;
  std::vector<hipEvent_t> raggedEvents;
  DevBuf stats;
  hipStream_t statsStream = nullptr;
  int statsState = 0;
  bool statsAccumulate = false;
  uint64_t statsHost[30] = { 0 };
  uint64_t statsPixels = 0;
  DevBuf lookback;
  DevBuf accTable;
  DevBuf devStatus;
  DevBuf in, planes;
  hipStream_t hostCopyStream = nullptr;
  hipStream_t hostStream = nullptr;
  std::vector<hipEvent_t> hostEvents;
  DevBuf hostWords;
  DevBuf cmp;
  DevBuf bFlags, bBound;
  DevBuf bOrder;
  DevBuf bMatch, bRegions, bOut, bPx, bFac, bNoise, bNoiseBase;
  HostBuf hFlags;
  HostBuf hRec, hBits, hDesc, hOut, hNoise, hNoiseBase;
  hipStream_t searchStream = nullptr;
  hipStream_t storeStream = nullptr;
  DevBuf bCalls;
  std::vector<hipEvent_t> workEvents;
  hipStream_t copyStream = nullptr;
  std::vector<hipEvent_t> bandEvents;
  std::vector<limg_hip::HostRegion> lastRegions;
  std::vector<uint32_t> regionPx;
  size_t lastBlocks = 0;
  double blockedMs[6] = { 0, 0, 0, 0, 0, 0 };
  double blockedKernelMs[4] = { 0, 0, 0, 0 };
  std::vector<hipEvent_t> workTimers;
  ncclComm_t comm = nullptr;
  int commRank = 0, commWorld = 1;
  const void *chainIn = nullptr;
  size_t chainX = 0, chainY = 0, chainBefore = 0;
  const void *chainFac[3] = { nullptr, nullptr, nullptr };
  int chainAlpha = 0, chainFast = 0;
  uint32_t chainEf = 0;
  DevBuf commWords;
  DevBuf streamFac, streamTiles, streamUnits, streamStatus, streamBuf;
  DevBuf bsUnits, bsTiles, bsMap, bsState;
  size_t blockedScratchCap = 0;
  struct { size_t sizeX = 0, sizeY = 0; int channels = 0; uint32_t errorFactor = 0, flags = 0; bool valid = false; } lastBlocked;
  std::vector<hipEvent_t> packTimers;
  bool packTimed = false;
  int persistentWorkgroups = 1280;
  bool forceSplit = false;
  bool profiling = false;
  std::vector<hipEvent_t> events;
  size_t eventsUsed = 0;

  template <class Ctx, class F>
  static void for_each_device_buffer(Ctx &c, F &&f)
  {
    for (auto *b : { &c.records, &c.shifts, &c.stripCalls, &c.stripBase, &c.invN, &c.noise, &c.noiseDyn, &c.noiseStates, &c.noiseCk, &c.park, &c.batchTable, &c.stats,
                     &c.lookback, &c.accTable, &c.devStatus, &c.in, &c.planes, &c.hostWords, &c.cmp, &c.bFlags, &c.bBound, &c.bOrder, &c.bMatch, &c.bRegions, &c.bOut,
                     &c.bPx, &c.bFac, &c.bNoise, &c.bNoiseBase, &c.bCalls, &c.commWords, &c.streamFac, &c.streamTiles, &c.streamUnits, &c.streamStatus, &c.streamBuf, &c.bsUnits, &c.bsTiles, &c.bsMap, &c.bsState })
      f(*b);
  }
};

namespace limg_hip
{
  uint64_t chain_call(uint64_t h, unsigned n, uint8_t *noise64, bool forceSoft, bool pcg);
  uint64_t fill_noise_table(uint64_t h, uint8_t *noise, size_t count, bool pcg);
  uint64_t chain_checkpoints(uint64_t h, size_t calls, size_t every, uint64_t *pOut, bool pcg);
  void chain_walk_rows(uint64_t &h, size_t &call, uint32_t by0, uint32_t by1, uint32_t blocksX, uint32_t stripsX, size_t sizeX, size_t sizeY, uint32_t chainCount, uint32_t chainRows,
                       const uint32_t *shifts, uint32_t *stripBase, unsigned long long *states, uint8_t *pixels, size_t maxCalls, bool pcg);
  size_t chain_walk_blocks(uint64_t h0, uint32_t blocksX, uint32_t blocksY, uint32_t stripsX, size_t sizeX, size_t sizeY, uint32_t chainCount, uint32_t chainRows, const uint32_t *shifts,
                           uint32_t *stripBase, unsigned long long *states, uint8_t *pixels, size_t maxCalls, bool pcg);

  size_t checkpoint_reach();
  bool dense_checkpoints_host(size_t first, size_t count, uint64_t *pOut);
  limg_hip_result ensure_checkpoints(limg_hip_context *c, size_t calls);
  limg_hip_result grow_noise_table(limg_hip_context *c, size_t entries, hipStream_t stream);
  bool chain_value_at(uint64_t calls, uint64_t *pValue);

  void mark(limg_hip_context *c, hipStream_t stream);

  template <class F>
  void run_on_threads(unsigned n, F &&work) noexcept
  {
    std::thread *pool = n > 1 ? new (std::nothrow) std::thread[n - 1] : nullptr;
    unsigned started = 0;
    if (pool)
      for (; started < n - 1; started++)
      {
        try { pool[started] = std::thread(work, started + 1); }
        catch (...) { break; }
      }
    work(0u);
    for (unsigned t = started + 1; t < n; t++) work(t);
    for (unsigned t = 0; t < started; t++) pool[t].join();
    delete[] pool;
  }

  struct Partition { uint32_t chainCount, chainRows; };
  Partition partition(size_t sizeY, int poolThreads);

  struct EncodeExtra
  {
    bool streamRaw = false, fitOnly = false;
    uint32_t *stripWords = nullptr;
    int chainPhase = 0;
    unsigned long long *dChainCalls = nullptr;
    const unsigned long long *dChainBase = nullptr;
    size_t chainBlocksBefore = 0;
    const ImageIO *batch = nullptr;
    size_t batchCount = 1;
    bool inner = false;
    int marks = 2;
    const Partition *part = nullptr;
    size_t scratchRow0 = 0;
    size_t scratchRows = 0;
    const unsigned long long *dPrevDesc = nullptr;
  };

  limg_hip_result encode_device(limg_hip_context *c, const uint32_t *dIn, size_t sizeX, size_t sizeY, int hasAlpha, const limg_hip_encode3d_info *dInfo,
                                const limg_hip_compact_out *compact, uint32_t errorFactor, int poolThreads, int fast, hipStream_t stream, const EncodeExtra &x = EncodeExtra());

  struct EncodeJob
  {
    limg_hip_context *c;
    hipStream_t stream;
    const EncodeExtra &x;
    const limg_hip_encode3d_info *dInfo;
    size_t sizeX, sizeY;
    EncodeParams p;
    Partition pt;
    int channels;
    bool ragged, fullPlanes, fused, wantStats;
    size_t blocks, strips;
    void mark_if(int level) const { if (x.marks >= level) mark(c, stream); }
  };
  limg_hip_result encode_stats(const EncodeJob &e);
  limg_hip_result encode_ragged(EncodeJob &e);

  limg_hip_result blocked_encode_device(limg_hip_context *c, const uint32_t *pIn, size_t sizeX, size_t sizeY, int hasAlpha, const limg_hip_blocked_encode3d_info *pInfo,
                                        uint32_t errorFactor, int fastBitCrushing, hipStream_t stream);
}

#endif
```

limg_amd/csrc/limg_hip_internal.h:

```cpp
#ifndef LIMG_HIP_INTERNAL_H
#define LIMG_HIP_INTERNAL_H

#include <hip/hip_runtime.h>
#include <stdint.h>

#include <type_traits>

#include "../../include/limg_hip.h"
#include "limg_hip_blocked_host.h"

namespace limg_hip
{
  constexpr int kBlock = 8;
  constexpr int kStripBlocks = 32;
  constexpr int kThreads = 256;
  constexpr int kWaves = 4;
  constexpr int kBlocksPerWave = 8;
  constexpr uint64_t kDitherSeed = 0xCA7F00D15BADF00DULL;

  struct ImageIO
  {
    const uint32_t *in;
    limg_hip_encode3d_info info;
  };

  struct EncodeParams
  {
    ImageIO io;
    const ImageIO *batch;
    uint32_t batchCount, imageStrips;
    uint32_t sizeX, sizeY, blocksX, blocksY, stripsX;
    uint32_t maxPixel32;
    uint64_t maxBlock;
    uint32_t blockLimitFull;
    int32_t crushBits, fast;
    const uint32_t *accTable;
    int32_t forced[3];
    int32_t recordLimit;
    uint32_t chainCount, chainRows;
    limg_hip_block_record *records;
    float *invN;
    uint32_t *shifts;
    uint32_t *stripCalls;
    uint32_t *stripBase;
    uint32_t *stripWords;
    int32_t storePlanes;
    int32_t fullPlanes;
    const uint8_t *noise;
    uint32_t noiseLast;
    unsigned long long *desc;
    uint32_t *ticket;
    int32_t zeroLookback;
    uint32_t *timeout;
#ifdef LIMG_HIP_TEST_HOOKS
    uint32_t lookbackSpins;
    uint32_t testBaseErrStrip;
    uint32_t testSkipStrip;
#endif
    uint8_t *park;
    int32_t compactOut;
    int32_t streamRaw;
    int32_t fitOnly;
    unsigned long long *chainCallsOut;
    const unsigned long long *chainBase;
    int32_t fitPrio;
    int32_t prefit;
    int32_t floatFast;
    int32_t vecIn;
    int32_t vecPlanes;
    int32_t vecFactors;
    int32_t vecFactors8;
    int32_t vecDecoded;
  };

  struct StreamParams
  {
    uint32_t sizeX, sizeY, blocksX, blocksY, nBlocks, nTiles, channels, errorFactor, flags;
    const uint8_t *fac[3];
    const limg_hip_block_record *records;
    const uint32_t *shifts;
    uint8_t *stream;
    uint32_t *tileBase;
    uint32_t *stripWords;
    uint32_t stripsX, nStrips, nWaves;
  };

  struct DecodeParams
  {
    uint32_t sizeX, sizeY, blocksX, blocksY, nBlocks;
    const uint8_t *stream;
    unsigned long long streamBytes;
    uint32_t *out;
    uint32_t *status;
    uint32_t *sink;
  };

  const uint64_t *noise_checkpoints_host(size_t *pCount, size_t *pEvery);
  const uint64_t *noise_checkpoints_far_host(size_t *pCount, size_t *pEvery);
  void launch_noise_fill(uint8_t *noise, const uint64_t *dCheckpoints, size_t count, hipStream_t s);
  void launch_noise_expand(uint8_t *noise, const unsigned long long *dStates, const uint8_t *dPixels, size_t calls, bool pcg, hipStream_t s);
  void launch_noise_expand_calls(uint8_t *noise, const unsigned long long *dStates, const unsigned long long *dOffsets, const uint32_t *dPixels, size_t calls, bool pcg, hipStream_t s);
  void launch_set_batch_table(ImageIO *dTable, const ImageIO *hTable, size_t count, hipStream_t s);
  template <class F> void with_flags(F &&f) { f(); }
  template <class F, class... Flags> void with_flags(F &&f, bool flag, Flags... rest)
  {
    if (!flag) with_flags([&](auto... b) { f(std::false_type(), b...); }, rest...);
    else with_flags([&](auto... b) { f(std::true_type(), b...); }, rest...);
  }

  void launch_fit_tpb(const EncodeParams &p, int channels, hipStream_t s);
  void launch_fit_search(const EncodeParams &p, int channels, hipStream_t s);
  void launch_encode_persistent(const EncodeParams &p, int channels, int workgroups, hipStream_t s);
  void launch_strip_scan(const EncodeParams &p, hipStream_t s);
  void launch_dither_store(const EncodeParams &p, int channels, hipStream_t s);
  void launch_shift_stats(const uint32_t *dShifts, uint32_t blocksX, uint32_t blocksY, uint32_t rows, uint32_t sizeX, uint32_t sizeY, unsigned long long *dOut30, hipStream_t s);
  void launch_chain_base(const unsigned long long *dCalls, int rank, int world, unsigned long long *dBase, uint32_t *dAborted, hipStream_t s);

  struct RegionDesc
  {
    uint32_t ox, oy, rx, ry;
    uint32_t keep;
    uint32_t scratch;
    uint32_t pad[2];
  };
  struct RegionOut
  {
    limg_hip_block_record rec;
    uint32_t shiftWord;
    uint32_t pad[3];
  };
  struct BlockedParams
  {
    const uint32_t *in;
    uint32_t sizeX, sizeY, blocksX, blocksY, channels;
    uint32_t maxPixel32;
    uint64_t maxBlock;
    int32_t crushBits, fast, forced[3];
    const limg_hip_block_record *pass1;
    unsigned long long *matchBits;
    uint32_t seedBase, seedCount;
    uint8_t *matchFlags;
    float *matchBound;
    const RegionDesc *regions;
    uint32_t nRegions;
    uint32_t regionBase;
    RegionOut *out;
    int32_t vecStore;
    uint32_t *order;
    uint32_t *scratchPx;
    uint8_t *scratchFac;
    uint32_t scratchCap;
    const uint8_t *noise;
    const unsigned long long *noiseBase;
    limg_hip_blocked_encode3d_info info;
  };

  void launch_blocked_bounds(const BlockedParams &p, hipStream_t s);
  void launch_blocked_match(const BlockedParams &p, hipStream_t s);
  void launch_blocked_fit_search(const BlockedParams &p, hipStream_t s);
  void launch_blocked_store(const BlockedParams &p, hipStream_t s);
  void launch_blocked_order(const BlockedParams &p, hipStream_t s);

  struct BlockedStreamParams
  {
    uint32_t sizeX, sizeY, blocksX, blocksY, channels, errorFactor, flags;
    uint32_t nRegions, nTiles, scratchCap;
    const RegionDesc *regions;
    const RegionOut *out;
    const unsigned long long *noiseBase;
    const uint8_t *scratchFac, *noise;
    uint8_t *stream;
    uint32_t *units;
    uint32_t *tiles;
  };
  struct BlockedDecodeParams
  {
    uint32_t sizeX, sizeY, blocksX, blocksY, nBlocks;
    const uint8_t *stream;
    unsigned long long streamBytes;
    uint32_t *out;
    uint32_t *map;
    uint32_t *status;
    uint32_t *state;
  };
  void launch_blocked_stream_pack(const BlockedStreamParams &p, int cus, hipStream_t s);
  void launch_blocked_stream_decode(const BlockedDecodeParams &p, int cus, hipStream_t s);

  struct WindowDecodeParams
  {
    uint32_t sizeX, sizeY, blocksX, blocksY, nBlocks;
    const uint8_t *stream;
    unsigned long long streamBytes;
    uint32_t x0, y0, width, height;
    uint32_t bx0, by0, wbx, wby;
    uint32_t *out;
    unsigned long long outStride;
    uint32_t vecOut;
    uint32_t *map;
    uint32_t *status;
    uint32_t *state;
  };
  void launch_stream_window_decode(const WindowDecodeParams &p, int cus, hipStream_t s);
  void launch_blocked_stream_window_decode(const WindowDecodeParams &p, int cus, hipStream_t s);

  void launch_stream_pack(const StreamParams &p, hipStream_t s);
  void launch_stream_decode(const DecodeParams &p, int cus, hipStream_t s);

  void launch_synth_random_gradient(uint32_t *out, uint32_t w, uint32_t h, uint64_t seed, int opaque, uint32_t y0, hipStream_t s);
  void launch_synth_photo_noise(uint32_t *out, uint32_t w, uint32_t h, uint64_t seed, uint32_t y0, hipStream_t s);
  void launch_compare(const uint32_t *a, const uint32_t *b, uint64_t count, int channels, unsigned long long *dErrorSum, hipStream_t s);
}

#endif
```

limg_amd/csrc/limg_hip_noise.cpp:

```cpp
#include <stdint.h>
#include <string.h>
#include <stddef.h>

#include <mutex>

#if defined(__x86_64__)
#include <immintrin.h>
#endif

namespace limg_hip
{
  namespace
  {
    const uint8_t kInvSbox[256] = {
      0x52, 0x09, 0x6a, 0xd5, 0x30, 0x36, 0xa5, 0x38, 0xbf, 0x40, 0xa3, 0x9e, 0x81, 0xf3, 0xd7, 0xfb, 0x7c, 0xe3, 0x39, 0x82, 0x9b, 0x2f, 0xff, 0x87, 0x34, 0x8e, 0x43, 0x44, 0xc4, 0xde, 0xe9, 0xcb,
      0x54, 0x7b, 0x94, 0x32, 0xa6, 0xc2, 0x23, 0x3d, 0xee, 0x4c, 0x95, 0x0b, 0x42, 0xfa, 0xc3, 0x4e, 0x08, 0x2e, 0xa1, 0x66, 0x28, 0xd9, 0x24, 0xb2, 0x76, 0x5b, 0xa2, 0x49, 0x6d, 0x8b, 0xd1, 0x25,
      0x72, 0xf8, 0xf6, 0x64, 0x86, 0x68, 0x98, 0x16, 0xd4, 0xa4, 0x5c, 0xcc, 0x5d, 0x65, 0xb6, 0x92, 0x6c, 0x70, 0x48, 0x50, 0xfd, 0xed, 0xb9, 0xda, 0x5e, 0x15, 0x46, 0x57, 0xa7, 0x8d, 0x9d, 0x84,
      0x90, 0xd8, 0xab, 0x00, 0x8c, 0xbc, 0xd3, 0x0a, 0xf7, 0xe4, 0x58, 0x05, 0xb8, 0xb3, 0x45, 0x06, 0xd0, 0x2c, 0x1e, 0x8f, 0xca, 0x3f, 0x0f, 0x02, 0xc1, 0xaf, 0xbd, 0x03, 0x01, 0x13, 0x8a, 0x6b,
      0x3a, 0x91, 0x11, 0x41, 0x4f, 0x67, 0xdc, 0xea, 0x97, 0xf2, 0xcf, 0xce, 0xf0, 0xb4, 0xe6, 0x73, 0x96, 0xac, 0x74, 0x22, 0xe7, 0xad, 0x35, 0x85, 0xe2, 0xf9, 0x37, 0xe8, 0x1c, 0x75, 0xdf, 0x6e,
      0x47, 0xf1, 0x1a, 0x71, 0x1d, 0x29, 0xc5, 0x89, 0x6f, 0xb7, 0x62, 0x0e, 0xaa, 0x18, 0xbe, 0x1b, 0xfc, 0x56, 0x3e, 0x4b, 0xc6, 0xd2, 0x79, 0x20, 0x9a, 0xdb, 0xc0, 0xfe, 0x78, 0xcd, 0x5a, 0xf4,
      0x1f, 0xdd, 0xa8, 0x33, 0x88, 0x07, 0xc7, 0x31, 0xb1, 0x12, 0x10, 0x59, 0x27, 0x80, 0xec, 0x5f, 0x60, 0x51, 0x7f, 0xa9, 0x19, 0xb5, 0x4a, 0x0d, 0x2d, 0xe5, 0x7a, 0x9f, 0x93, 0xc9, 0x9c, 0xef,
      0xa0, 0xe0, 0x3b, 0x4d, 0xae, 0x2a, 0xf5, 0xb0, 0xc8, 0xeb, 0xbb, 0x3c, 0x83, 0x53, 0x99, 0x61, 0x17, 0x2b, 0x04, 0x7e, 0xba, 0x77, 0xd6, 0x26, 0xe1, 0x69, 0x14, 0x63, 0x55, 0x21, 0x0c, 0x7d
    };

    const uint32_t kKey[4] = { 0xAB705E1Du, 0x824A73EAu, 0x06CB4CADu, 0x2A76E980u };

    uint32_t g_td[4][256];
    bool g_td_ready = false;

    inline uint8_t xtime(uint8_t x) { return (uint8_t)((x << 1) ^ ((x >> 7) * 0x1B)); }

    void build_tables_once()
    {
      for (int x = 0; x < 256; x++)
      {
        const uint8_t s = kInvSbox[x];
        const uint8_t s2 = xtime(s), s4 = xtime(s2), s8 = xtime(s4);
        const uint8_t m9 = (uint8_t)(s8 ^ s), m11 = (uint8_t)(s8 ^ s2 ^ s), m13 = (uint8_t)(s8 ^ s4 ^ s), m14 = (uint8_t)(s8 ^ s4 ^ s2);
        g_td[0][x] = (uint32_t)m14 | ((uint32_t)m9 << 8) | ((uint32_t)m13 << 16) | ((uint32_t)m11 << 24);
        g_td[1][x] = (uint32_t)m11 | ((uint32_t)m14 << 8) | ((uint32_t)m9 << 16) | ((uint32_t)m13 << 24);
        g_td[2][x] = (uint32_t)m13 | ((uint32_t)m11 << 8) | ((uint32_t)m14 << 16) | ((uint32_t)m9 << 24);
        g_td[3][x] = (uint32_t)m9 | ((uint32_t)m13 << 8) | ((uint32_t)m11 << 16) | ((uint32_t)m14 << 24);
      }
      g_td_ready = true;
    }

    void build_tables()
    {
      static std::once_flag once;
      std::call_once(once, build_tables_once);
    }

    inline void aesdec_soft(uint32_t st[4])
    {
      uint32_t o[4];
      for (int c = 0; c < 4; c++)
      {
        o[c] = g_td[0][st[c] & 0xFF] ^ g_td[1][(st[(c + 3) & 3] >> 8) & 0xFF] ^ g_td[2][(st[(c + 2) & 3] >> 16) & 0xFF] ^ g_td[3][(st[(c + 1) & 3] >> 24) & 0xFF] ^ kKey[c];
      }
      memcpy(st, o, 16);
    }

#if defined(__x86_64__)
    __attribute__((target("aes,sse4.1"))) void walk_aesni(uint64_t &h, unsigned rounds, uint8_t *noise)
    {
      const __m128i key = _mm_set_epi64x(0x2A76E98006CB4CADLL, (long long)0x824A73EAAB705E1DULL);
      const __m128i pick = _mm_set_epi8(-1, -1, -1, -1, -1, -1, -1, -1, 14, 12, 10, 8, 6, 4, 2, 0);
      __m128i st = _mm_set_epi64x((long long)~h, (long long)h);
      unsigned j = 0;
      if (noise && rounds >= 64 && (reinterpret_cast<uintptr_t>(noise) & 7u) == 0)
      {
        for (; j < rounds && (reinterpret_cast<uintptr_t>(noise + 8 * j) & 63u); j++)
        {
          st = _mm_aesdec_si128(st, key);
          _mm_storel_epi64(reinterpret_cast<__m128i *>(noise + 8 * j), _mm_shuffle_epi8(st, pick));
        }
        for (; j + 8 <= rounds; j += 8)
        {
          __m128i *line = reinterpret_cast<__m128i *>(noise + 8 * j);
          for (int k = 0; k < 4; k++)
          {
            st = _mm_aesdec_si128(st, key);
            const __m128i lo = _mm_shuffle_epi8(st, pick);
            st = _mm_aesdec_si128(st, key);
            _mm_stream_si128(line + k, _mm_unpacklo_epi64(lo, _mm_shuffle_epi8(st, pick)));
          }
        }
        _mm_sfence();
      }
      for (; j < rounds; j++)
      {
        st = _mm_aesdec_si128(st, key);
        if (noise) _mm_storel_epi64(reinterpret_cast<__m128i *>(noise + 8 * j), _mm_shuffle_epi8(st, pick));
      }
      h = (uint64_t)_mm_cvtsi128_si64(st);
    }
#endif

    void walk_soft(uint64_t &h, unsigned rounds, uint8_t *noise)
    {
      build_tables();
      uint32_t st[4];
      const uint64_t inv = ~h;
      memcpy(st, &h, 8);
      memcpy(st + 2, &inv, 8);
      for (unsigned j = 0; j < rounds; j++)
      {
        aesdec_soft(st);
        if (noise)
          for (int i = 0; i < 8; i++) noise[8 * j + i] = (uint8_t)(st[i >> 1] >> (16 * (i & 1)));
      }
      memcpy(&h, st, 8);
    }

    bool have_aesni()
    {
#if defined(__x86_64__)
      static const bool v = __builtin_cpu_supports("aes") && __builtin_cpu_supports("sse4.1");
      return v;
#else
      return false;
#endif
    }

    inline uint32_t pcg_step(uint64_t &h)
    {
      h = h * 6364136223846793005ULL + 1;
      const uint32_t xorshifted_hi = (uint32_t)(((h >> 18) ^ h) >> 27);
      const uint32_t rot_hi = (uint32_t)(h >> 59);
      return (xorshifted_hi >> rot_hi) | (xorshifted_hi << ((uint32_t)(-(int32_t)rot_hi) & 31));
    }
  }

  uint64_t chain_call(uint64_t h, unsigned n, uint8_t *noise64, bool forceSoft, bool pcg)
  {
    const unsigned rounds = (!pcg && n >= 8) ? n / 8 : 0;
    if (rounds)
    {
#if defined(__x86_64__)
      if (have_aesni() && !forceSoft) walk_aesni(h, rounds, noise64);
      else
#endif
        walk_soft(h, rounds, noise64);
    }
    for (unsigned i = rounds * 8; i < n; i++)
    {
      const uint32_t r = pcg_step(h);
      if (noise64) noise64[i] = (uint8_t)r;
    }
    return h;
  }

#if defined(__x86_64__)
  __attribute__((target("aes,sse4.1"))) static uint64_t walk_batch_aesni(uint64_t h, size_t count, const uint8_t *shiftWords, size_t stride, const uint32_t *npx,
                                                                        unsigned long long *noiseBase, unsigned long long *callState, unsigned long long *callOff,
                                                                        uint32_t *callPx, uint64_t &noiseOff, size_t &callCount, size_t maxCalls)
  {
    const __m128i key = _mm_set_epi64x(0x2A76E98006CB4CADLL, (long long)0x824A73EAAB705E1DULL);
    for (size_t i = 0; i < count; i++)
    {
      noiseBase[i] = noiseOff;
      uint32_t word;
      memcpy(&word, shiftWords + i * stride, 4);
      const uint32_t calls = word >> 24, n = npx[i], rounds = n >= 8 ? n / 8 : 0, tail = n - rounds * 8;
      for (uint32_t k = 0; k < calls && callCount < maxCalls; k++, noiseOff += n, callCount++)
      {
        callState[callCount] = h; callOff[callCount] = noiseOff; callPx[callCount] = n;
        if (rounds)
        {
          __m128i st = _mm_set_epi64x((long long)~h, (long long)h);
          for (uint32_t j = 0; j < rounds; j++) st = _mm_aesdec_si128(st, key);
          h = (uint64_t)_mm_cvtsi128_si64(st);
        }
        for (uint32_t j = 0; j < tail; j++) (void)pcg_step(h);
      }
    }
    return h;
  }
#endif

  namespace
  {
    template <bool NI>
#if defined(__x86_64__)
    __attribute__((target("aes,sse4.1")))
#endif
    void walk_blocks_impl(uint64_t &hIo, size_t &callIo, uint32_t by0, uint32_t by1, uint32_t blocksX, uint32_t stripsX, size_t sizeX, size_t sizeY, uint32_t chainCount, uint32_t chainRows,
                          const uint32_t *shifts, uint32_t *stripBase, unsigned long long *states, uint8_t *pixels, size_t maxCalls, bool pcg)
    {
#if defined(__x86_64__)
      const __m128i key = _mm_set_epi64x(0x2A76E98006CB4CADLL, (long long)0x824A73EAAB705E1DULL);
#endif
      auto chain_of = [&](uint32_t row) -> uint32_t { if (chainCount <= 1 || chainRows == 0) return 0u; const uint32_t c = row / chainRows; return c < chainCount - 1 ? c : chainCount - 1; };
      uint64_t h = hIo;
      size_t call = callIo;
      for (uint32_t by = by0; by < by1; by++)
      {
        if (by != 0 && chain_of(by) != chain_of(by - 1)) h = 0xCA7F00D15BADF00DULL;
        const unsigned ry = (unsigned)((sizeY - (size_t)by * 8) < 8 ? (sizeY - (size_t)by * 8) : 8);
        for (uint32_t bx = 0; bx < blocksX; bx++)
        {
          if (bx % 32u == 0) stripBase[(size_t)by * stripsX + bx / 32u] = (uint32_t)call;
          const unsigned rx = (unsigned)((sizeX - (size_t)bx * 8) < 8 ? (sizeX - (size_t)bx * 8) : 8);
          const uint32_t n = rx * ry, calls = shifts[(size_t)by * blocksX + bx] >> 24, rounds = (!pcg && n >= 8) ? n / 8 : 0, tail = n - rounds * 8;
          for (uint32_t k = 0; k < calls && call < maxCalls; k++, call++)
          {
            states[call] = h; pixels[call] = (uint8_t)n;
            if (NI)
            {
#if defined(__x86_64__)
              if (rounds)
              {
                __m128i st = _mm_set_epi64x((long long)~h, (long long)h);
                for (uint32_t j = 0; j < rounds; j++) st = _mm_aesdec_si128(st, key);
                h = (uint64_t)_mm_cvtsi128_si64(st);
              }
              for (uint32_t j = 0; j < tail; j++) (void)pcg_step(h);
#endif
            }
            else h = chain_call(h, n, nullptr, false, pcg);
          }
        }
      }
      hIo = h; callIo = call;
    }
  }

  void chain_walk_rows(uint64_t &h, size_t &call, uint32_t by0, uint32_t by1, uint32_t blocksX, uint32_t stripsX, size_t sizeX, size_t sizeY, uint32_t chainCount, uint32_t chainRows,
                       const uint32_t *shifts, uint32_t *stripBase, unsigned long long *states, uint8_t *pixels, size_t maxCalls, bool pcg)
  {
#if defined(__x86_64__)
    if (!pcg && have_aesni()) { walk_blocks_impl<true>(h, call, by0, by1, blocksX, stripsX, sizeX, sizeY, chainCount, chainRows, shifts, stripBase, states, pixels, maxCalls, pcg); return; }
#endif
    walk_blocks_impl<false>(h, call, by0, by1, blocksX, stripsX, sizeX, sizeY, chainCount, chainRows, shifts, stripBase, states, pixels, maxCalls, pcg);
  }

  size_t chain_walk_blocks(uint64_t h0, uint32_t blocksX, uint32_t blocksY, uint32_t stripsX, size_t sizeX, size_t sizeY, uint32_t chainCount, uint32_t chainRows, const uint32_t *shifts,
                           uint32_t *stripBase, unsigned long long *states, uint8_t *pixels, size_t maxCalls, bool pcg)
  {
    uint64_t h = h0;
    size_t call = 0;
    chain_walk_rows(h, call, 0, blocksY, blocksX, stripsX, sizeX, sizeY, chainCount, chainRows, shifts, stripBase, states, pixels, maxCalls, pcg);
    return call;
  }

  uint64_t chain_walk_batch(uint64_t h, size_t count, const uint8_t *shiftWords, size_t stride, const uint32_t *npx, unsigned long long *noiseBase, unsigned long long *callState,
                            unsigned long long *callOff, uint32_t *callPx, uint64_t &noiseOff, size_t &callCount, size_t maxCalls, bool pcg)
  {
#if defined(__x86_64__)
    if (!pcg && have_aesni()) return walk_batch_aesni(h, count, shiftWords, stride, npx, noiseBase, callState, callOff, callPx, noiseOff, callCount, maxCalls);
#endif
    for (size_t i = 0; i < count; i++)
    {
      noiseBase[i] = noiseOff;
      uint32_t word;
      memcpy(&word, shiftWords + i * stride, 4);
      const uint32_t calls = word >> 24;
      for (uint32_t k = 0; k < calls && callCount < maxCalls; k++, noiseOff += npx[i], callCount++)
      {
        callState[callCount] = h; callOff[callCount] = noiseOff; callPx[callCount] = npx[i];
        h = chain_call(h, npx[i], nullptr, false, pcg);
      }
    }
    return h;
  }

  uint64_t chain_checkpoints(uint64_t h, size_t calls, size_t every, uint64_t *pOut, bool pcg)
  {
    for (size_t k = 0; k < calls; k++)
    {
      if (pOut && every && k % every == 0) pOut[k / every] = h;
      h = chain_call(h, 64, nullptr, false, pcg);
    }
    return h;
  }

  uint64_t fill_noise_table(uint64_t h, uint8_t *noise, size_t count, bool pcg)
  {
    for (size_t k = 0; k < count; k++) h = chain_call(h, 64, noise + k * 64, false, pcg);
    return h;
  }
}
```

limg_amd/csrc/limg_hip_noise_gpu.hip:

```cpp
#include "limg_hip_internal.h"
#include "limg_noise_checkpoints.h"

namespace limg_hip
{
  namespace
  {
    __constant__ uint8_t d_inv_sbox[256] = {
      0x52, 0x09, 0x6a, 0xd5, 0x30, 0x36, 0xa5, 0x38, 0xbf, 0x40, 0xa3, 0x9e, 0x81, 0xf3, 0xd7, 0xfb, 0x7c, 0xe3, 0x39, 0x82, 0x9b, 0x2f, 0xff, 0x87, 0x34, 0x8e, 0x43, 0x44, 0xc4, 0xde, 0xe9, 0xcb,
      0x54, 0x7b, 0x94, 0x32, 0xa6, 0xc2, 0x23, 0x3d, 0xee, 0x4c, 0x95, 0x0b, 0x42, 0xfa, 0xc3, 0x4e, 0x08, 0x2e, 0xa1, 0x66, 0x28, 0xd9, 0x24, 0xb2, 0x76, 0x5b, 0xa2, 0x49, 0x6d, 0x8b, 0xd1, 0x25,
      0x72, 0xf8, 0xf6, 0x64, 0x86, 0x68, 0x98, 0x16, 0xd4, 0xa4, 0x5c, 0xcc, 0x5d, 0x65, 0xb6, 0x92, 0x6c, 0x70, 0x48, 0x50, 0xfd, 0xed, 0xb9, 0xda, 0x5e, 0x15, 0x46, 0x57, 0xa7, 0x8d, 0x9d, 0x84,
      0x90, 0xd8, 0xab, 0x00, 0x8c, 0xbc, 0xd3, 0x0a, 0xf7, 0xe4, 0x58, 0x05, 0xb8, 0xb3, 0x45, 0x06, 0xd0, 0x2c, 0x1e, 0x8f, 0xca, 0x3f, 0x0f, 0x02, 0xc1, 0xaf, 0xbd, 0x03, 0x01, 0x13, 0x8a, 0x6b,
      0x3a, 0x91, 0x11, 0x41, 0x4f, 0x67, 0xdc, 0xea, 0x97, 0xf2, 0xcf, 0xce, 0xf0, 0xb4, 0xe6, 0x73, 0x96, 0xac, 0x74, 0x22, 0xe7, 0xad, 0x35, 0x85, 0xe2, 0xf9, 0x37, 0xe8, 0x1c, 0x75, 0xdf, 0x6e,
      0x47, 0xf1, 0x1a, 0x71, 0x1d, 0x29, 0xc5, 0x89, 0x6f, 0xb7, 0x62, 0x0e, 0xaa, 0x18, 0xbe, 0x1b, 0xfc, 0x56, 0x3e, 0x4b, 0xc6, 0xd2, 0x79, 0x20, 0x9a, 0xdb, 0xc0, 0xfe, 0x78, 0xcd, 0x5a, 0xf4,
      0x1f, 0xdd, 0xa8, 0x33, 0x88, 0x07, 0xc7, 0x31, 0xb1, 0x12, 0x10, 0x59, 0x27, 0x80, 0xec, 0x5f, 0x60, 0x51, 0x7f, 0xa9, 0x19, 0xb5, 0x4a, 0x0d, 0x2d, 0xe5, 0x7a, 0x9f, 0x93, 0xc9, 0x9c, 0xef,
      0xa0, 0xe0, 0x3b, 0x4d, 0xae, 0x2a, 0xf5, 0xb0, 0xc8, 0xeb, 0xbb, 0x3c, 0x83, 0x53, 0x99, 0x61, 0x17, 0x2b, 0x04, 0x7e, 0xba, 0x77, 0xd6, 0x26, 0xe1, 0x69, 0x14, 0x63, 0x55, 0x21, 0x0c, 0x7d
    };

    __device__ __forceinline__ uint32_t xtime(uint32_t x) { return ((x << 1) ^ ((x >> 7) * 0x1Bu)) & 0xFFu; }

    __global__ __launch_bounds__(64) void k_noise_fill(uint8_t *noise, const uint64_t *checkpoints, uint32_t segments, uint64_t count)
    {
      __shared__ uint32_t td[4][256];
      for (uint32_t x = threadIdx.x; x < 256; x += 64)
      {
        const uint32_t s = d_inv_sbox[x], s2 = xtime(s), s4 = xtime(s2), s8 = xtime(s4);
        const uint32_t m9 = s8 ^ s, m11 = s8 ^ s2 ^ s, m13 = s8 ^ s4 ^ s, m14 = s8 ^ s4 ^ s2;
        td[0][x] = m14 | (m9 << 8) | (m13 << 16) | (m11 << 24);
        td[1][x] = m11 | (m14 << 8) | (m9 << 16) | (m13 << 24);
        td[2][x] = m13 | (m11 << 8) | (m14 << 16) | (m9 << 24);
        td[3][x] = m9 | (m13 << 8) | (m11 << 16) | (m14 << 24);
      }
      __syncthreads();
      const uint32_t seg = blockIdx.x * 64u + threadIdx.x;
      if (seg >= segments) return;
      const uint32_t key[4] = { 0xAB705E1Du, 0x824A73EAu, 0x06CB4CADu, 0x2A76E980u };
      unsigned long long h = checkpoints[seg];
      const uint64_t first = (uint64_t)seg * LIMG_NOISE_CHECKPOINT_EVERY;
      const uint64_t n = min((uint64_t)LIMG_NOISE_CHECKPOINT_EVERY, count - first);
      uint4 *out = reinterpret_cast<uint4 *>(noise + first * 64);
      for (uint64_t k = 0; k < n; k++)
      {
        uint32_t st[4] = { (uint32_t)h, (uint32_t)(h >> 32), ~(uint32_t)h, ~(uint32_t)(h >> 32) };
        uint32_t bytes[16];
#pragma unroll
        for (int j = 0; j < 8; j++)
        {
          uint32_t o[4];
#pragma unroll
          for (int c = 0; c < 4; c++)
            o[c] = td[0][st[c] & 0xFFu] ^ td[1][(st[(c + 3) & 3] >> 8) & 0xFFu] ^ td[2][(st[(c + 2) & 3] >> 16) & 0xFFu] ^ td[3][st[(c + 1) & 3] >> 24] ^ key[c];
#pragma unroll
          for (int c = 0; c < 4; c++) st[c] = o[c];
          bytes[2 * j] = __builtin_amdgcn_perm(st[1], st[0], 0x06040200u);
          bytes[2 * j + 1] = __builtin_amdgcn_perm(st[3], st[2], 0x06040200u);
        }
#pragma unroll
        for (int q = 0; q < 4; q++) out[k * 4 + q] = make_uint4(bytes[4 * q], bytes[4 * q + 1], bytes[4 * q + 2], bytes[4 * q + 3]);
        h = (unsigned long long)st[0] | ((unsigned long long)st[1] << 32);
      }
    }
  }

  namespace
  {
    __global__ __launch_bounds__(256) void k_noise_expand(uint8_t *noise, const unsigned long long *states, const uint8_t *pixels, uint32_t calls, int pcg)
    {
      __shared__ uint32_t td[4][256];
      for (uint32_t x = threadIdx.x; x < 256; x += 256)
      {
        const uint32_t s = d_inv_sbox[x], s2 = xtime(s), s4 = xtime(s2), s8 = xtime(s4);
        const uint32_t m9 = s8 ^ s, m11 = s8 ^ s2 ^ s, m13 = s8 ^ s4 ^ s, m14 = s8 ^ s4 ^ s2;
        td[0][x] = m14 | (m9 << 8) | (m13 << 16) | (m11 << 24);
        td[1][x] = m11 | (m14 << 8) | (m9 << 16) | (m13 << 24);
        td[2][x] = m13 | (m11 << 8) | (m14 << 16) | (m9 << 24);
        td[3][x] = m9 | (m13 << 8) | (m11 << 16) | (m14 << 24);
      }
      __syncthreads();
      const uint32_t k = blockIdx.x * 256u + threadIdx.x;
      if (k >= calls) return;
      const uint32_t key[4] = { 0xAB705E1Du, 0x824A73EAu, 0x06CB4CADu, 0x2A76E980u };
      unsigned long long h = states[k];
      const uint32_t n = pixels[k], rounds = (!pcg && n >= 8u) ? n / 8u : 0u;
      uint32_t bytes[16];
#pragma unroll
      for (int i = 0; i < 16; i++) bytes[i] = 0u;
      uint32_t st[4] = { (uint32_t)h, (uint32_t)(h >> 32), ~(uint32_t)h, ~(uint32_t)(h >> 32) };
#pragma unroll
      for (int j = 0; j < 8; j++)
      {
        if ((uint32_t)j < rounds)
        {
          uint32_t o[4];
#pragma unroll
          for (int c = 0; c < 4; c++)
            o[c] = td[0][st[c] & 0xFFu] ^ td[1][(st[(c + 3) & 3] >> 8) & 0xFFu] ^ td[2][(st[(c + 2) & 3] >> 16) & 0xFFu] ^ td[3][st[(c + 1) & 3] >> 24] ^ key[c];
#pragma unroll
          for (int c = 0; c < 4; c++) st[c] = o[c];
          bytes[2 * j] = __builtin_amdgcn_perm(st[1], st[0], 0x06040200u);
          bytes[2 * j + 1] = __builtin_amdgcn_perm(st[3], st[2], 0x06040200u);
        }
      }
      if (rounds) h = (unsigned long long)st[0] | ((unsigned long long)st[1] << 32);
      uint4 *out = reinterpret_cast<uint4 *>(noise + (size_t)k * 64);
#pragma unroll
      for (int q = 0; q < 4; q++) out[q] = make_uint4(bytes[4 * q], bytes[4 * q + 1], bytes[4 * q + 2], bytes[4 * q + 3]);
      for (uint32_t i = rounds * 8u; i < n; i++)
      {
        h = h * 6364136223846793005ULL + 1ULL;
        const uint32_t xs = (uint32_t)(((h >> 18) ^ h) >> 27), rot = (uint32_t)(h >> 59);
        noise[(size_t)k * 64 + i] = (uint8_t)((xs >> rot) | (xs << ((0u - rot) & 31u)));
      }
    }
  }

  namespace
  {
    __global__ __launch_bounds__(256) void k_noise_expand_calls(uint8_t *noise, const unsigned long long *states, const unsigned long long *offsets, const uint32_t *pixels,
                                                               uint32_t calls, int pcg)
    {
      __shared__ uint32_t td[4][256];
      {
        const uint32_t x = threadIdx.x;
        const uint32_t s = d_inv_sbox[x], s2 = xtime(s), s4 = xtime(s2), s8 = xtime(s4);
        const uint32_t m9 = s8 ^ s, m11 = s8 ^ s2 ^ s, m13 = s8 ^ s4 ^ s, m14 = s8 ^ s4 ^ s2;
        td[0][x] = m14 | (m9 << 8) | (m13 << 16) | (m11 << 24);
        td[1][x] = m11 | (m14 << 8) | (m9 << 16) | (m13 << 24);
        td[2][x] = m13 | (m11 << 8) | (m14 << 16) | (m9 << 24);
        td[3][x] = m9 | (m13 << 8) | (m11 << 16) | (m14 << 24);
      }
      __syncthreads();
      const uint32_t k = blockIdx.x * 256u + threadIdx.x;
      if (k >= calls) return;
      const uint32_t key[4] = { 0xAB705E1Du, 0x824A73EAu, 0x06CB4CADu, 0x2A76E980u };
      unsigned long long h = states[k];
      const uint32_t n = pixels[k], rounds = (!pcg && n >= 8u) ? n / 8u : 0u;
      uint8_t *out = noise + offsets[k];
      uint32_t st[4] = { (uint32_t)h, (uint32_t)(h >> 32), ~(uint32_t)h, ~(uint32_t)(h >> 32) };
      const bool aligned = (reinterpret_cast<uintptr_t>(out) & 7u) == 0;
      for (uint32_t j = 0; j < rounds; j++)
      {
        uint32_t o[4];
#pragma unroll
        for (int c = 0; c < 4; c++)
          o[c] = td[0][st[c] & 0xFFu] ^ td[1][(st[(c + 3) & 3] >> 8) & 0xFFu] ^ td[2][(st[(c + 2) & 3] >> 16) & 0xFFu] ^ td[3][st[(c + 1) & 3] >> 24] ^ key[c];
#pragma unroll
        for (int c = 0; c < 4; c++) st[c] = o[c];
        const uint32_t lo = __builtin_amdgcn_perm(st[1], st[0], 0x06040200u), hi = __builtin_amdgcn_perm(st[3], st[2], 0x06040200u);
        if (aligned) *reinterpret_cast<uint2 *>(out + 8 * (size_t)j) = make_uint2(lo, hi);
        else
        {
#pragma unroll
          for (int b = 0; b < 4; b++) { out[8 * (size_t)j + b] = (uint8_t)(lo >> (8 * b)); out[8 * (size_t)j + 4 + b] = (uint8_t)(hi >> (8 * b)); }
        }
      }
      if (rounds) h = (unsigned long long)st[0] | ((unsigned long long)st[1] << 32);
      for (uint32_t i = rounds * 8u; i < n; i++)
      {
        h = h * 6364136223846793005ULL + 1ULL;
        const uint32_t xs = (uint32_t)(((h >> 18) ^ h) >> 27), rot = (uint32_t)(h >> 59);
        out[i] = (uint8_t)((xs >> rot) | (xs << ((0u - rot) & 31u)));
      }
    }
  }

  void launch_noise_expand_calls(uint8_t *noise, const unsigned long long *dStates, const unsigned long long *dOffsets, const uint32_t *dPixels, size_t calls, bool pcg, hipStream_t s)
  {
    if (calls == 0) return;
    hipLaunchKernelGGL(k_noise_expand_calls, dim3((uint32_t)((calls + 255u) / 256u)), dim3(256), 0, s, noise, dStates, dOffsets, dPixels, (uint32_t)calls, pcg ? 1 : 0);
  }

  void launch_noise_expand(uint8_t *noise, const unsigned long long *dStates, const uint8_t *dPixels, size_t calls, bool pcg, hipStream_t s)
  {
    if (calls == 0) return;
    hipLaunchKernelGGL(k_noise_expand, dim3((uint32_t)((calls + 255u) / 256u)), dim3(256), 0, s, noise, dStates, dPixels, (uint32_t)calls, pcg ? 1 : 0);
  }

  const uint64_t *noise_checkpoints_host(size_t *pCount, size_t *pEvery)
  {
    static const uint64_t table[LIMG_NOISE_CHECKPOINT_COUNT] = LIMG_NOISE_CHECKPOINTS_INIT;
    if (pCount) *pCount = LIMG_NOISE_CHECKPOINT_COUNT;
    if (pEvery) *pEvery = LIMG_NOISE_CHECKPOINT_EVERY;
    return table;
  }

  const uint64_t *noise_checkpoints_far_host(size_t *pCount, size_t *pEvery)
  {
    static const uint64_t table[LIMG_NOISE_FAR_COUNT] = LIMG_NOISE_FAR_INIT;
    if (pCount) *pCount = LIMG_NOISE_FAR_COUNT;
    if (pEvery) *pEvery = LIMG_NOISE_FAR_EVERY;
    return table;
  }

  void launch_noise_fill(uint8_t *noise, const uint64_t *dCheckpoints, size_t count, hipStream_t s)
  {
    const uint32_t segments = (uint32_t)((count + LIMG_NOISE_CHECKPOINT_EVERY - 1) / LIMG_NOISE_CHECKPOINT_EVERY);
    if (segments == 0) return;
    hipLaunchKernelGGL(k_noise_fill, dim3((segments + 63u) / 64u), dim3(64), 0, s, noise, dCheckpoints, segments, (uint64_t)count);
  }
}
```

Before: 50830.

## Parallelize blocked store per 8x8 block and split noise expansion into segments

Replaces the per-region vectorized store kernel (one wave per region looping over pixels) with a per-8x8-block kernel. Each 8-lane group handles one block; a new prefix-sum kernel over region block counts plus a binary search map work units to regions. The noise expansion now carries the full AES state per fixed-length segment, so long calls are split across many threads instead of serialized in one. This targets load imbalance from large regions and long noise calls, at the cost of an extra single-workgroup prefix launch, more host-side segment records, and a stricter 8-byte alignment requirement for the vector path.

```diff
diff --git a/limg_amd/csrc/limg_hip_blocked.hip b/limg_amd/csrc/limg_hip_blocked.hip
--- a/limg_amd/csrc/limg_hip_blocked.hip
+++ b/limg_amd/csrc/limg_hip_blocked.hip
@@ -640,6 +640,203 @@
       }
     }
 
+    __global__ __launch_bounds__(1024) void k_blocked_block_prefix(const BlockedParams p)
+    {
+      __shared__ uint32_t sWave[16];
+      __shared__ uint32_t sCarry;
+      const int tid = threadIdx.x, lane = lane_id(), wave = tid >> 6;
+      const uint32_t n = p.nRegions;
+      if (tid == 0) sCarry = 0;
+      __syncthreads();
+      for (uint32_t base = 0; base < n; base += 4096)
+      {
+        const uint32_t i0 = base + (uint32_t)tid * 4u;
+        uint32_t nb[4], sum = 0;
+#pragma unroll
+        for (int k = 0; k < 4; k++)
+        {
+          nb[k] = 0;
+          if (i0 + k < n) { const RegionDesc &R = p.regions[p.order ? p.order[i0 + k] : i0 + k]; nb[k] = R.rx * R.ry; }
+          sum += nb[k];
+        }
+        const uint32_t incl = wave_scan_inclusive(sum, lane);
+        if (lane == 63) sWave[wave] = incl;
+        __syncthreads();
+        uint32_t before = sCarry + incl - sum;
+        for (int w = 0; w < wave; w++) before += sWave[w];
+#pragma unroll
+        for (int k = 0; k < 4; k++)
+        {
+          if (i0 + k < n) p.blockPrefix[i0 + k] = before;
+          before += nb[k];
+        }
+        __syncthreads();
+        if (tid == 0)
+        {
+          uint32_t t = sCarry;
+          for (int w = 0; w < 16; w++) t += sWave[w];
+          sCarry = t;
+        }
+        __syncthreads();
+      }
+    }
+
+    typedef uint32_t u32x2_a4 __attribute__((ext_vector_type(2), aligned(4)));
+
+    constexpr bool kStoreUnitsNonTemporal = false;
+    typedef uint32_t u32x4_t __attribute__((ext_vector_type(4)));
+    typedef uint32_t u32x2_t __attribute__((ext_vector_type(2)));
+    __device__ __forceinline__ void store_plane(void *dst, uint4 v)
+    {
+      if (kStoreUnitsNonTemporal) __builtin_nontemporal_store(u32x4_t{ v.x, v.y, v.z, v.w }, reinterpret_cast<u32x4_t *>(dst));
+      else *reinterpret_cast<uint4 *>(dst) = v;
+    }
+    __device__ __forceinline__ void store_plane(void *dst, uint2 v)
+    {
+      if (kStoreUnitsNonTemporal) __builtin_nontemporal_store(u32x2_t{ v.x, v.y }, reinterpret_cast<u32x2_t *>(dst));
+      else *reinterpret_cast<uint2 *>(dst) = v;
+    }
+
+    template <int CH>
+    __global__ __launch_bounds__(256) void k_blocked_store_units(const BlockedParams p)
+    {
+      const int lane = lane_id(), b = lane >> 3, t = lane & 7;
+      const uint32_t unit = (uint32_t)__builtin_amdgcn_readfirstlane((int)(blockIdx.x * 4u + (threadIdx.x >> 6)));
+      const uint32_t total = p.nBatchBlocks, nR = p.nRegions, B0 = unit * 8u;
+      if (B0 >= total) return;
+      const uint32_t *prefix = p.blockPrefix;
+      uint32_t lo = 0, hi = min(nR, B0 + 1u);
+      while (hi - lo > 1u)
+      {
+        const uint32_t mid = (lo + hi) >> 1;
+        if (prefix[mid] <= B0) lo = mid; else hi = mid;
+      }
+      const uint32_t B = B0 + (uint32_t)b, ei = lo + 1u + (uint32_t)t;
+      const uint32_t e = ei < nR ? prefix[ei] : 0xFFFFFFFFu;
+      const unsigned long long le = __builtin_amdgcn_ballot_w64(e <= B);
+      if (B >= total) return;
+      const uint32_t j = lo + (uint32_t)__builtin_popcount((uint32_t)(le >> (8 * b)) & 0xFFu);
+      const uint32_t r = p.order ? p.order[j] : j;
+      const uint32_t q = B - prefix[j];
+      const RegionDesc R = p.regions[r];
+      const RegionOut O = p.out[r];
+      const limg_hip_block_record &rec = O.rec;
+      const uint32_t shift[3] = { O.shiftWord & 0xFF, (O.shiftWord >> 8) & 0xFF, (O.shiftWord >> 16) & 0xFF };
+      const uint32_t n = R.rx * R.ry * (uint32_t)(kBlock * kBlock), xpx = R.rx * kBlock, cap = p.scratchCap;
+      const uint32_t by = q / R.rx, bx = q - by * R.rx;
+      const uint32_t i = (by * kBlock + (uint32_t)t) * xpx + bx * kBlock;
+      const size_t oBlock = (size_t)(R.oy + by) * kBlock * p.sizeX + (size_t)(R.ox + bx) * kBlock;
+      const size_t oRow = oBlock + (size_t)t * p.sizeX;
+      const size_t o1 = oBlock + (size_t)(t & ~1) * p.sizeX + (size_t)(t & 1) * 4u, o2 = o1 + p.sizeX;
+      const uint8_t *sf = p.scratchFac + R.scratch;
+
+      const int16_t *vec[6] = { rec.dirA_min, rec.dirA_max, rec.dirB_offset, rec.dirB_mag, rec.dirC_offset, rec.dirC_mag };
+      uint32_t col[6];
+#pragma unroll
+      for (int k = 0; k < 6; k++)
+      {
+        uint32_t v = 0;
+#pragma unroll
+        for (int c = 0; c < CH; c++)
+        {
+          int w = (int)vec[k][c] + (k >= 2 ? 0x80 : 0);
+          w = w < 0 ? 0 : (w > 255 ? 255 : w);
+          v |= (uint32_t)w << (8 * c);
+        }
+        if (CH == 3) v |= 0xFF000000u;
+        col[k] = v;
+      }
+      const uint32_t pa = shift[0] == 8 ? 0xFFu : shift[0] * 0x22u, pb = shift[1] == 8 ? 0xFFu : shift[1] * 0x22u, pc = shift[2] == 8 ? 0xFFu : shift[2] * 0x22u;
+      const uint32_t shiftVal = 0xFF000000u | (pa << 16) | (pb << 8) | pc;
+      const uint32_t perPixel = (8 - shift[0]) + (8 - shift[1]) + (8 - shift[2]);
+      const uint8_t bpp = (uint8_t)(perPixel + ((uint32_t)(CH * 18 + CH * 8 + 32) + n / 2) / n);
+      const uint32_t blockIndex = 0xFF000000u | (p.regionBase + r + 1u);
+      int nn[3][4], mc[3][4];
+#pragma unroll
+      for (int f = 0; f < 3; f++)
+#pragma unroll
+        for (int c = 0; c < 4; c++)
+        {
+          int nv = (int)vec[2 * f + 1][c] - (int)vec[2 * f][c], m = (int)vec[2 * f][c];
+          if (c < 3) { if (shift[f] > 7) { nv = 0; if (f > 0) m = 0; } }
+          else if (CH == 3) { nv = 0; m = 0xFFFF; }
+          nn[f][c] = nv;
+          mc[f][c] = (int)(((uint32_t)m << 8) + 128u);
+        }
+      const int mul[3] = { (int)shift_mul(shift[0]), (int)shift_mul(shift[1]), (int)shift_mul(shift[2]) };
+
+      uint32_t fq[3][2];
+      {
+        const uint8_t *nz = p.noise + p.noiseBase[r];
+#pragma unroll
+        for (int k = 0; k < 3; k++)
+        {
+          const u32x2_a4 f8 = *reinterpret_cast<const u32x2_a4 *>(sf + (size_t)k * cap + i);
+          fq[k][0] = f8.x; fq[k][1] = f8.y;
+          const uint32_t s = shift[k];
+          if (s != 0 && s != 8)
+          {
+            const uint2 z8 = *reinterpret_cast<const uint2 *>(nz + i);
+            const uint32_t z[2] = { z8.x, z8.y };
+#pragma unroll
+            for (int h = 0; h < 2; h++)
+            {
+              uint32_t out = 0;
+#pragma unroll
+              for (int x = 0; x < 4; x++)
+              {
+                int v = (int)((fq[k][h] >> (8 * x)) & 0xFFu) + ((int)((z[h] >> (8 * x)) & ((1u << s) - 1u)) - (int)(1u << (s - 1)));
+                v = v < 0 ? 0 : (v > 255 ? 255 : v);
+                out |= ((uint32_t)v >> s) << (8 * x);
+              }
+              fq[k][h] = out;
+            }
+            nz += n;
+          }
+        }
+      }
+      uint8_t *const facPlane[3] = { p.info.pFactorsA, p.info.pFactorsB, p.info.pFactorsC };
+#pragma unroll
+      for (int k = 0; k < 3; k++)
+      {
+        const uint32_t keep = ((0xFFu << shift[k]) & 0xFFu) * 0x01010101u;
+        const uint2 v = shift[k] > 7 ? make_uint2(0u, 0u) : make_uint2((fq[k][0] << shift[k]) & keep, (fq[k][1] << shift[k]) & keep);
+        store_plane(facPlane[k] + oRow, v);
+      }
+      store_plane(p.info.pBitsPerPixel + oRow, make_uint2((uint32_t)bpp * 0x01010101u, (uint32_t)bpp * 0x01010101u));
+      uint32_t *const uniPlane[8] = { p.info.pShiftABCX, p.info.pColAMin, p.info.pColAMax, p.info.pColBMin, p.info.pColBMax, p.info.pColCMin, p.info.pColCMax, p.info.pBlockIndex };
+      const uint32_t uniVal[8] = { shiftVal, col[0], col[1], col[2], col[3], col[4], col[5], blockIndex };
+#pragma unroll
+      for (int k = 0; k < 8; k++)
+      {
+        const uint4 v = make_uint4(uniVal[k], uniVal[k], uniVal[k], uniVal[k]);
+        store_plane(uniPlane[k] + o1, v);
+        store_plane(uniPlane[k] + o2, v);
+      }
+      uint32_t dec[8];
+#pragma unroll
+      for (int x = 0; x < 8; x++)
+      {
+        const int dA = (int)((fq[0][x >> 2] >> (8 * (x & 3))) & 0xFFu) * mul[0], dB = (int)((fq[1][x >> 2] >> (8 * (x & 3))) & 0xFFu) * mul[1],
+                  dC = (int)((fq[2][x >> 2] >> (8 * (x & 3))) & 0xFFu) * mul[2];
+        uint32_t decoded = 0;
+#pragma unroll
+        for (int c = 0; c < 4; c++)
+        {
+          int est = (mad_i24(dA, nn[0][c], mc[0][c]) >> 8) + (mad_i24(dB, nn[1][c], mc[1][c]) >> 8) + (mad_i24(dC, nn[2][c], mc[2][c]) >> 8);
+          est = est < 0 ? 0 : (est > 255 ? 255 : est);
+          decoded |= (uint32_t)est << (8 * c);
+        }
+        dec[x] = decoded;
+      }
+      const bool odd = (t & 1) != 0;
+      uint32_t got[4];
+#pragma unroll
+      for (int x = 0; x < 4; x++) got[x] = (uint32_t)dpp<0xB1, 0xF>(0, (int)(odd ? dec[x] : dec[4 + x]));
+      store_plane(p.info.pDecoded + o1, odd ? make_uint4(got[0], got[1], got[2], got[3]) : make_uint4(dec[0], dec[1], dec[2], dec[3]));
+      store_plane(p.info.pDecoded + o2, odd ? make_uint4(dec[4], dec[5], dec[6], dec[7]) : make_uint4(got[0], got[1], got[2], got[3]));
+    }
+
     template <int CH>
     __global__ __launch_bounds__(64) void k_blocked_store(const BlockedParams p)
     {
@@ -698,69 +895,6 @@
         }
       }
 
-      if (p.vecStore)
-      {
-        for (uint32_t base = 0; base < n; base += 256)
-        {
-          const uint32_t i = base + (uint32_t)lane * 4u;
-          if (i >= n) continue;
-          const uint32_t row = i / g.xpx, colx = i - row * g.xpx;
-          const size_t o = (size_t)(g.py0 + row) * p.sizeX + g.px0 + colx;
-          uint32_t fq[3];
-#pragma unroll
-          for (int k = 0; k < 3; k++)
-          {
-            uint32_t f4 = *reinterpret_cast<const uint32_t *>(sf + (size_t)k * cap + i);
-            const uint32_t s = shift[k];
-            if (s != 0 && s != 8)
-            {
-              const uint32_t z4 = *reinterpret_cast<const uint32_t *>(nz[k] + i);
-              uint32_t out = 0;
-#pragma unroll
-              for (int q = 0; q < 4; q++)
-              {
-                int t = (int)((f4 >> (8 * q)) & 0xFFu) + ((int)((z4 >> (8 * q)) & ((1u << s) - 1u)) - (int)(1u << (s - 1)));
-                t = t < 0 ? 0 : (t > 255 ? 255 : t);
-                out |= ((uint32_t)t >> s) << (8 * q);
-              }
-              f4 = out;
-            }
-            fq[k] = f4;
-          }
-          uint32_t st[3];
-#pragma unroll
-          for (int k = 0; k < 3; k++) st[k] = shift[k] > 7 ? 0u : ((fq[k] << shift[k]) & ((0xFFu << shift[k]) & 0xFFu) * 0x01010101u);
-          *reinterpret_cast<uint32_t *>(p.info.pFactorsA + o) = st[0];
-          *reinterpret_cast<uint32_t *>(p.info.pFactorsB + o) = st[1];
-          *reinterpret_cast<uint32_t *>(p.info.pFactorsC + o) = st[2];
-          *reinterpret_cast<uint32_t *>(p.info.pBitsPerPixel + o) = (uint32_t)bpp * 0x01010101u;
-          *reinterpret_cast<uint4 *>(p.info.pShiftABCX + o) = make_uint4(shiftVal, shiftVal, shiftVal, shiftVal);
-          *reinterpret_cast<uint4 *>(p.info.pColAMin + o) = make_uint4(col[0], col[0], col[0], col[0]);
-          *reinterpret_cast<uint4 *>(p.info.pColAMax + o) = make_uint4(col[1], col[1], col[1], col[1]);
-          *reinterpret_cast<uint4 *>(p.info.pColBMin + o) = make_uint4(col[2], col[2], col[2], col[2]);
-          *reinterpret_cast<uint4 *>(p.info.pColBMax + o) = make_uint4(col[3], col[3], col[3], col[3]);
-          *reinterpret_cast<uint4 *>(p.info.pColCMin + o) = make_uint4(col[4], col[4], col[4], col[4]);
-          *reinterpret_cast<uint4 *>(p.info.pColCMax + o) = make_uint4(col[5], col[5], col[5], col[5]);
-          *reinterpret_cast<uint4 *>(p.info.pBlockIndex + o) = make_uint4(blockIndex, blockIndex, blockIndex, blockIndex);
-          uint32_t dec[4];
-#pragma unroll
-          for (int q = 0; q < 4; q++)
-          {
-            const int dA = (int)((fq[0] >> (8 * q)) & 0xFFu) * mulA, dB = (int)((fq[1] >> (8 * q)) & 0xFFu) * mulB, dC = (int)((fq[2] >> (8 * q)) & 0xFFu) * mulC;
-            uint32_t decoded = 0;
-#pragma unroll
-            for (int c = 0; c < 4; c++)
-            {
-              int est = (mad_i24(dA, nn[0][c], mc[0][c]) >> 8) + (mad_i24(dB, nn[1][c], mc[1][c]) >> 8) + (mad_i24(dC, nn[2][c], mc[2][c]) >> 8);
-              est = est < 0 ? 0 : (est > 255 ? 255 : est);
-              decoded |= (uint32_t)est << (8 * c);
-            }
-            dec[q] = decoded;
-          }
-          *reinterpret_cast<uint4 *>(p.info.pDecoded + o) = make_uint4(dec[0], dec[1], dec[2], dec[3]);
-        }
-        return;
-      }
       for (uint32_t base = 0; base < n; base += 64)
       {
         const uint32_t i = base + lane;
@@ -832,9 +966,22 @@
     hipLaunchKernelGGL(k_blocked_order, dim3(1), dim3(1024), 0, s, p);
   }
 
+  void launch_blocked_block_prefix(const BlockedParams &p, hipStream_t s)
+  {
+    if (p.nRegions == 0 || !p.vecStore) return;
+    hipLaunchKernelGGL(k_blocked_block_prefix, dim3(1), dim3(1024), 0, s, p);
+  }
+
   void launch_blocked_store(const BlockedParams &p, hipStream_t s)
   {
     if (p.nRegions == 0) return;
+    if (p.vecStore)
+    {
+      const dim3 grid((p.nBatchBlocks + 31u) / 32u), block(256);
+      if (p.channels == 4) hipLaunchKernelGGL(k_blocked_store_units<4>, grid, block, 0, s, p);
+      else hipLaunchKernelGGL(k_blocked_store_units<3>, grid, block, 0, s, p);
+      return;
+    }
     if (p.channels == 4) hipLaunchKernelGGL(k_blocked_store<4>, dim3(p.nRegions), dim3(64), 0, s, p);
     else hipLaunchKernelGGL(k_blocked_store<3>, dim3(p.nRegions), dim3(64), 0, s, p);
   }
diff --git a/limg_amd/csrc/limg_hip_blocked_api.hip b/limg_amd/csrc/limg_hip_blocked_api.hip
--- a/limg_amd/csrc/limg_hip_blocked_api.hip
+++ b/limg_amd/csrc/limg_hip_blocked_api.hip
@@ -34,7 +34,7 @@
   {
     limg_hip_context *c;
     hipStream_t s;
-    size_t sizeX, sizeY, blocks, maxCalls;
+    size_t sizeX, sizeY, blocks, maxSegments;
     uint32_t blocksX, blocksY, bandRows, nBands;
     int channels; bool pcg;
     bool compact;
@@ -42,9 +42,9 @@
     hipEvent_t *frontTimers;
     limg_hip_block_record *hRec; unsigned long long *hBits; uint8_t *hFlags;
     RegionDesc *desc; RegionOut *hOut; unsigned long long *noiseBase;
-    unsigned long long *callState, *callOff, *dCallState, *dCallOff;
-    uint32_t *callPx, *dCallPx;
+    NoiseSegment *segments, *dSegments;
     uint32_t *npx;
+    uint32_t *blocksTo;
   };
 
   limg_hip_result set_up(BlockedJob &j, limg_hip_context *c, const uint32_t *pIn, size_t sizeX, size_t sizeY, int hasAlpha, const limg_hip_blocked_encode3d_info &info,
@@ -53,7 +53,8 @@
     j.compact = compact;
     j.c = c; j.s = (hipStream_t)stream; j.sizeX = sizeX; j.sizeY = sizeY; j.channels = hasAlpha ? 4 : 3; j.pcg = c->opt.dither_pcg != 0;
     j.blocksX = (uint32_t)((sizeX + kBlock - 1) / kBlock); j.blocksY = (uint32_t)((sizeY + kBlock - 1) / kBlock);
-    j.blocks = (size_t)j.blocksX * j.blocksY; j.maxCalls = 3 * j.blocks;
+    j.blocks = (size_t)j.blocksX * j.blocksY;
+    j.maxSegments = 3 * j.blocks;
     j.bandRows = (j.blocksY + kBands - 1) / kBands; j.nBands = (j.blocksY + j.bandRows - 1) / j.bandRows;
     const uint64_t capMax = ((uint64_t)sizeX * sizeY + 3ull * j.blocks + 3ull) & ~3ull;
     if (capMax > 0xFFFFFFF0ull) return limg_hip_error_InvalidParameter;
@@ -71,7 +72,7 @@
     bp.scratchCap = (uint32_t)capMax;
     uintptr_t w = 0, b8 = 0;
     for_each_written_plane([&](auto m) { (sizeof(*(info.*m)) == 4 ? w : b8) |= (uintptr_t)(info.*m); });
-    bp.vecStore = (sizeX % kBlock == 0 && sizeY % kBlock == 0 && (w & 15u) == 0 && (b8 & 3u) == 0 && TOPT(c, blocked_no_vec_store) == 0) ? 1 : 0;
+    bp.vecStore = (sizeX % kBlock == 0 && sizeY % kBlock == 0 && (w & 15u) == 0 && (b8 & 7u) == 0 && TOPT(c, blocked_no_vec_store) == 0) ? 1 : 0;
     return limg_hip_success;
   }
 
@@ -82,7 +83,7 @@
   limg_hip_result ensure_resources(BlockedJob &j)
   {
     limg_hip_context *c = j.c;
-    const size_t blocks = j.blocks, maxCalls = j.maxCalls, px = j.sizeX * j.sizeY, capMax = j.bp.scratchCap;
+    const size_t blocks = j.blocks, maxSegments = j.maxSegments, px = j.sizeX * j.sizeY, capMax = j.bp.scratchCap;
     const bool bound = TOPT(c, blocked_no_bound) == 0;
     limg_hip_result r = ensure_events(c->workTimers, 4 * kInFlight + 3, hipEventDefault);
     auto need = [&r](auto &buf, size_t bytes) { if (r == limg_hip_success) r = buf.ensure(bytes); };
@@ -91,21 +92,21 @@
     need(c->hRec, blocks * sizeof(limg_hip_block_record)); need(c->hBits, blocks * kMatchWords * 8);
     if (r == limg_hip_success) r = ensure_events(c->bandEvents, 2 * kBands + 1, hipEventDisableTiming);
     need(c->hDesc, blocks * sizeof(RegionDesc)); need(c->hOut, blocks * sizeof(RegionOut)); need(c->hNoiseBase, blocks * 8 + 8);
-    need(c->hNoise, maxCalls * 20 + 64); need(c->bCalls, maxCalls * 20 + 64);
+    need(c->hNoise, maxSegments * sizeof(NoiseSegment)); need(c->bCalls, maxSegments * sizeof(NoiseSegment));
     need(c->bRegions, blocks * sizeof(RegionDesc)); need(c->bOut, blocks * sizeof(RegionOut)); need(c->bNoiseBase, blocks * 8 + 8); need(c->bOrder, blocks * 4);
+    if (j.bp.vecStore) need(c->bBlockPrefix, blocks * 4);
     need(c->bNoise, 3 * px + 64); need(c->bPx, capMax * 4); need(c->bFac, capMax * 3);
     for (hipStream_t *st : { &c->copyStream, &c->searchStream, &c->storeStream })
       if (r == limg_hip_success) r = ensure_stream(*st);
     if (r == limg_hip_success) r = ensure_events(c->workEvents, kInFlight, hipEventDisableTiming);
     if (r != limg_hip_success) return r;
-    try { c->regionPx.resize(blocks); }
+    try { c->regionPx.resize(blocks); c->regionBlocksTo.resize(blocks + 1); }
     catch (const std::bad_alloc &) { return limg_hip_error_MemoryAllocationFailure; }
-    j.npx = c->regionPx.data();
+    j.npx = c->regionPx.data(); j.blocksTo = c->regionBlocksTo.data(); j.blocksTo[0] = 0;
     j.frontTimers = c->workTimers.data() + 4 * kInFlight;
     j.hRec = (limg_hip_block_record *)c->hRec.p; j.hBits = (unsigned long long *)c->hBits.p; j.hFlags = (uint8_t *)c->hFlags.p;
     j.desc = (RegionDesc *)c->hDesc.p; j.hOut = (RegionOut *)c->hOut.p; j.noiseBase = (unsigned long long *)c->hNoiseBase.p;
-    j.callState = (unsigned long long *)c->hNoise.p; j.callOff = j.callState + maxCalls; j.callPx = (uint32_t *)(j.callOff + maxCalls);
-    j.dCallState = (unsigned long long *)c->bCalls.p; j.dCallOff = j.dCallState + maxCalls; j.dCallPx = (uint32_t *)(j.dCallOff + maxCalls);
+    j.segments = (NoiseSegment *)c->hNoise.p; j.dSegments = (NoiseSegment *)c->bCalls.p;
     j.bp.matchBits = (unsigned long long *)c->bMatch.p; j.bp.matchFlags = (uint8_t *)c->bFlags.p;
     if (bound) j.bp.matchBound = (float *)c->bBound.p;
     j.bp.scratchPx = (uint32_t *)c->bPx.p; j.bp.scratchFac = (uint8_t *)c->bFac.p; j.bp.noise = (const uint8_t *)c->bNoise.p;
@@ -169,6 +170,7 @@
         if (h.oy + h.ry == j.blocksY && (j.sizeY % kBlock)) ypx = ypx - kBlock + j.sizeY % kBlock;
         j.npx[i] = (uint32_t)(xpx * ypx);
         j.desc[i] = { h.ox, h.oy, h.rx, h.ry, h.keep, (uint32_t)cap, { 0, 0 } };
+        j.blocksTo[i + 1] = j.blocksTo[i] + h.rx * h.ry;
         cap += ((uint64_t)j.npx[i] + 3) & ~3ull;
       }
       laid = count;
@@ -202,7 +204,7 @@
     Batch queue[kInFlight];
     size_t head = 0, tail = 0, issued = 0;
     bool fin = false;
-    uint64_t chain = kDitherSeed, noiseOff = 0; size_t callCount = 0;
+    uint64_t chain = kDitherSeed, noiseOff = 0; size_t segmentCount = 0;
     double kernelMs[2] = { 0, 0 };
     double busy[3] = { 0, 0, 0 };
     bool storeTimed[kInFlight] = {};
@@ -215,6 +217,7 @@
       q.regions = (const RegionDesc *)c->bRegions.p + b.r0; q.nRegions = (uint32_t)(b.r1 - b.r0); q.regionBase = (uint32_t)b.r0;
       q.out = (RegionOut *)c->bOut.p + b.r0; q.noiseBase = (const unsigned long long *)c->bNoiseBase.p + b.r0;
       q.order = (b.r1 - b.r0 >= kOrderFrom && TOPT(c, blocked_no_order) == 0) ? (uint32_t *)c->bOrder.p + b.r0 : nullptr;
+      if (q.vecStore) { q.blockPrefix = (uint32_t *)c->bBlockPrefix.p + b.r0; q.nBatchBlocks = j.blocksTo[b.r1] - j.blocksTo[b.r0]; }
       return q;
     }
     void enqueue_published(bool mayWait, size_t minNew)
@@ -253,28 +256,32 @@
       bool ok = hipEventSynchronize(c->workEvents[pending.ev]) == hipSuccess;
       if (ok) add_elapsed(kernelMs[0], c->workTimers[4 * pending.ev], c->workTimers[4 * pending.ev + 1]);
       const clk::time_point w1 = clk::now();
-      const size_t call0 = callCount;
+      const size_t seg0 = segmentCount;
       for (size_t w = pending.r0; ok && w < pending.r1; w += kWalkPiece)
       {
         const size_t n = pending.r1 - w < kWalkPiece ? pending.r1 - w : kWalkPiece;
-        chain = chain_walk_batch(chain, n, reinterpret_cast<const uint8_t *>(&j.hOut[w].shiftWord), sizeof(RegionOut), j.npx + w, j.noiseBase + w, j.callState, j.callOff,
-                                 j.callPx, noiseOff, callCount, j.maxCalls, j.pcg);
+        chain = chain_walk_batch(chain, n, reinterpret_cast<const uint8_t *>(&j.hOut[w].shiftWord), sizeof(RegionOut), j.npx + w, j.noiseBase + w, j.segments,
+                                 noiseOff, segmentCount, j.maxSegments, j.pcg);
         if (w + n < pending.r1) enqueue_published(false, kWorthFromInsideAWalk);
       }
       const clk::time_point w2 = clk::now();
-      const size_t nc = callCount - call0;
+      const size_t nc = segmentCount - seg0;
       const hipStream_t ss = c->storeStream;
       ok = ok && hipStreamWaitEvent(ss, c->workEvents[pending.ev], 0) == hipSuccess;
       ok = ok && hipEventRecord(c->workTimers[4 * pending.ev + 2], ss) == hipSuccess;
       if (ok && nc)
       {
-        ok = hipMemcpyAsync(j.dCallState + call0, j.callState + call0, nc * 8, hipMemcpyHostToDevice, ss) == hipSuccess &&
-             hipMemcpyAsync(j.dCallOff + call0, j.callOff + call0, nc * 8, hipMemcpyHostToDevice, ss) == hipSuccess &&
-             hipMemcpyAsync(j.dCallPx + call0, j.callPx + call0, nc * 4, hipMemcpyHostToDevice, ss) == hipSuccess;
-        if (ok) { launch_noise_expand_calls((uint8_t *)c->bNoise.p, j.dCallState + call0, j.dCallOff + call0, j.dCallPx + call0, nc, j.pcg, ss); ok = hipGetLastError() == hipSuccess; }
+        ok = hipMemcpyAsync(j.dSegments + seg0, j.segments + seg0, nc * sizeof(NoiseSegment), hipMemcpyHostToDevice, ss) == hipSuccess;
+        if (ok) { launch_noise_expand_segments((uint8_t *)c->bNoise.p, j.dSegments + seg0, nc, j.pcg, ss); ok = hipGetLastError() == hipSuccess; }
       }
       ok = ok && hipMemcpyAsync((unsigned long long *)c->bNoiseBase.p + pending.r0, j.noiseBase + pending.r0, (pending.r1 - pending.r0) * 8, hipMemcpyHostToDevice, ss) == hipSuccess;
-      if (ok && !j.compact) { launch_blocked_store(params_of(pending), ss); ok = hipGetLastError() == hipSuccess; }
+      if (ok && !j.compact)
+      {
+        const BlockedParams q = params_of(pending);
+        launch_blocked_block_prefix(q, ss);
+        launch_blocked_store(q, ss);
+        ok = hipGetLastError() == hipSuccess;
+      }
       if (ok && hipEventRecord(c->workTimers[4 * pending.ev + 3], ss) == hipSuccess) storeTimed[pending.ev] = true;
       const clk::time_point w3 = clk::now();
       busy[0] += ms(w0, w1); busy[1] += ms(w1, w2); busy[2] += ms(w2, w3);
diff --git a/limg_amd/csrc/limg_hip_blocked_host.h b/limg_amd/csrc/limg_hip_blocked_host.h
--- a/limg_amd/csrc/limg_hip_blocked_host.h
+++ b/limg_amd/csrc/limg_hip_blocked_host.h
@@ -22,8 +22,10 @@
                      const std::function<void(size_t)> *progress = nullptr, const std::function<void(uint32_t)> *needSeedRow = nullptr, const uint8_t *seedFlags = nullptr,
                      const std::function<void()> *needRecords = nullptr);
   bool blocked_matches_host(int channels, const limg_hip_block_record &seed, const limg_hip_block_record &cand);
-  uint64_t chain_walk_batch(uint64_t h, size_t count, const uint8_t *shiftWords, size_t stride, const uint32_t *npx, unsigned long long *noiseBase, unsigned long long *callState,
-                            unsigned long long *callOff, uint32_t *callPx, uint64_t &noiseOff, size_t &callCount, size_t maxCalls, bool pcg);
+  constexpr uint32_t kNoiseSegmentRounds = 64;
+  struct NoiseSegment { uint64_t lo, hi, offset; uint32_t px, pad; };
+  uint64_t chain_walk_batch(uint64_t h, size_t count, const uint8_t *shiftWords, size_t stride, const uint32_t *npx, unsigned long long *noiseBase, NoiseSegment *segments,
+                            uint64_t &noiseOff, size_t &segmentCount, size_t maxSegments, bool pcg);
 }
 
 #endif
diff --git a/limg_amd/csrc/limg_hip_context.h b/limg_amd/csrc/limg_hip_context.h
--- a/limg_amd/csrc/limg_hip_context.h
+++ b/limg_amd/csrc/limg_hip_context.h
@@ -106,6 +106,7 @@
   DevBuf cmp;
   DevBuf bFlags, bBound;
   DevBuf bOrder;
+  DevBuf bBlockPrefix;
   DevBuf bMatch, bRegions, bOut, bPx, bFac, bNoise, bNoiseBase;
   HostBuf hFlags;
   HostBuf hRec, hBits, hDesc, hOut, hNoise, hNoiseBase;
@@ -117,6 +118,7 @@
   std::vector<hipEvent_t> bandEvents;
   std::vector<limg_hip::HostRegion> lastRegions;
   std::vector<uint32_t> regionPx;
+  std::vector<uint32_t> regionBlocksTo;
   size_t lastBlocks = 0;
   double blockedMs[6] = { 0, 0, 0, 0, 0, 0 };
   double blockedKernelMs[4] = { 0, 0, 0, 0 };
@@ -145,7 +147,7 @@
   static void for_each_device_buffer(Ctx &c, F &&f)
   {
     for (auto *b : { &c.records, &c.shifts, &c.stripCalls, &c.stripBase, &c.invN, &c.noise, &c.noiseDyn, &c.noiseStates, &c.noiseCk, &c.park, &c.batchTable, &c.stats,
-                     &c.lookback, &c.accTable, &c.devStatus, &c.in, &c.planes, &c.hostWords, &c.cmp, &c.bFlags, &c.bBound, &c.bOrder, &c.bMatch, &c.bRegions, &c.bOut,
+                     &c.lookback, &c.accTable, &c.devStatus, &c.in, &c.planes, &c.hostWords, &c.cmp, &c.bFlags, &c.bBound, &c.bOrder, &c.bBlockPrefix, &c.bMatch, &c.bRegions, &c.bOut,
                      &c.bPx, &c.bFac, &c.bNoise, &c.bNoiseBase, &c.bCalls, &c.commWords, &c.streamFac, &c.streamTiles, &c.streamUnits, &c.streamStatus, &c.streamBuf, &c.bsUnits, &c.bsTiles, &c.bsMap, &c.bsState })
       f(*b);
   }
diff --git a/limg_amd/csrc/limg_hip_internal.h b/limg_amd/csrc/limg_hip_internal.h
--- a/limg_amd/csrc/limg_hip_internal.h
+++ b/limg_amd/csrc/limg_hip_internal.h
@@ -99,7 +99,7 @@
   const uint64_t *noise_checkpoints_far_host(size_t *pCount, size_t *pEvery);
   void launch_noise_fill(uint8_t *noise, const uint64_t *dCheckpoints, size_t count, hipStream_t s);
   void launch_noise_expand(uint8_t *noise, const unsigned long long *dStates, const uint8_t *dPixels, size_t calls, bool pcg, hipStream_t s);
-  void launch_noise_expand_calls(uint8_t *noise, const unsigned long long *dStates, const unsigned long long *dOffsets, const uint32_t *dPixels, size_t calls, bool pcg, hipStream_t s);
+  void launch_noise_expand_segments(uint8_t *noise, const NoiseSegment *dSegments, size_t segments, bool pcg, hipStream_t s);
   void launch_set_batch_table(ImageIO *dTable, const ImageIO *hTable, size_t count, hipStream_t s);
   template <class F> void with_flags(F &&f) { f(); }
   template <class F, class... Flags> void with_flags(F &&f, bool flag, Flags... rest)
@@ -147,6 +147,8 @@
     RegionOut *out;
     int32_t vecStore;
     uint32_t *order;
+    uint32_t *blockPrefix;
+    uint32_t nBatchBlocks;
     uint32_t *scratchPx;
     uint8_t *scratchFac;
     uint32_t scratchCap;
@@ -160,6 +162,7 @@
   void launch_blocked_fit_search(const BlockedParams &p, hipStream_t s);
   void launch_blocked_store(const BlockedParams &p, hipStream_t s);
   void launch_blocked_order(const BlockedParams &p, hipStream_t s);
+  void launch_blocked_block_prefix(const BlockedParams &p, hipStream_t s);
 
   struct BlockedStreamParams
   {
diff --git a/limg_amd/csrc/limg_hip_noise.cpp b/limg_amd/csrc/limg_hip_noise.cpp
--- a/limg_amd/csrc/limg_hip_noise.cpp
+++ b/limg_amd/csrc/limg_hip_noise.cpp
@@ -3,6 +3,8 @@
 #include <stddef.h>
 
 #include <mutex>
+
+#include "limg_hip_blocked_host.h"
 
 #if defined(__x86_64__)
 #include <immintrin.h>
@@ -153,8 +155,8 @@
 
 #if defined(__x86_64__)
   __attribute__((target("aes,sse4.1"))) static uint64_t walk_batch_aesni(uint64_t h, size_t count, const uint8_t *shiftWords, size_t stride, const uint32_t *npx,
-                                                                        unsigned long long *noiseBase, unsigned long long *callState, unsigned long long *callOff,
-                                                                        uint32_t *callPx, uint64_t &noiseOff, size_t &callCount, size_t maxCalls)
+                                                                        unsigned long long *noiseBase, NoiseSegment *segments, uint64_t &noiseOff, size_t &segmentCount,
+                                                                        size_t maxSegments)
   {
     const __m128i key = _mm_set_epi64x(0x2A76E98006CB4CADLL, (long long)0x824A73EAAB705E1DULL);
     for (size_t i = 0; i < count; i++)
@@ -163,15 +165,23 @@
       uint32_t word;
       memcpy(&word, shiftWords + i * stride, 4);
       const uint32_t calls = word >> 24, n = npx[i], rounds = n >= 8 ? n / 8 : 0, tail = n - rounds * 8;
-      for (uint32_t k = 0; k < calls && callCount < maxCalls; k++, noiseOff += n, callCount++)
-      {
-        callState[callCount] = h; callOff[callCount] = noiseOff; callPx[callCount] = n;
-        if (rounds)
-        {
-          __m128i st = _mm_set_epi64x((long long)~h, (long long)h);
-          for (uint32_t j = 0; j < rounds; j++) st = _mm_aesdec_si128(st, key);
-          h = (uint64_t)_mm_cvtsi128_si64(st);
-        }
+      for (uint32_t k = 0; k < calls; k++, noiseOff += n)
+      {
+        __m128i st = _mm_set_epi64x((long long)~h, (long long)h);
+        uint32_t done = 0;
+        do
+        {
+          const uint32_t r = rounds - done < kNoiseSegmentRounds ? rounds - done : kNoiseSegmentRounds;
+          if (segmentCount < maxSegments)
+          {
+            NoiseSegment *seg = segments + segmentCount++;
+            _mm_storeu_si128(reinterpret_cast<__m128i *>(seg), st);
+            seg->offset = noiseOff + 8ull * done; seg->px = 8u * r + (done + r == rounds ? tail : 0u); seg->pad = 0;
+          }
+          for (uint32_t j = 0; j < r; j++) st = _mm_aesdec_si128(st, key);
+          done += r;
+        } while (done < rounds);
+        if (rounds) h = (uint64_t)_mm_cvtsi128_si64(st);
         for (uint32_t j = 0; j < tail; j++) (void)pcg_step(h);
       }
     }
@@ -244,22 +254,40 @@
     return call;
   }
 
-  uint64_t chain_walk_batch(uint64_t h, size_t count, const uint8_t *shiftWords, size_t stride, const uint32_t *npx, unsigned long long *noiseBase, unsigned long long *callState,
-                            unsigned long long *callOff, uint32_t *callPx, uint64_t &noiseOff, size_t &callCount, size_t maxCalls, bool pcg)
-  {
-#if defined(__x86_64__)
-    if (!pcg && have_aesni()) return walk_batch_aesni(h, count, shiftWords, stride, npx, noiseBase, callState, callOff, callPx, noiseOff, callCount, maxCalls);
-#endif
+  uint64_t chain_walk_batch(uint64_t h, size_t count, const uint8_t *shiftWords, size_t stride, const uint32_t *npx, unsigned long long *noiseBase, NoiseSegment *segments,
+                            uint64_t &noiseOff, size_t &segmentCount, size_t maxSegments, bool pcg)
+  {
+#if defined(__x86_64__)
+    if (!pcg && have_aesni()) return walk_batch_aesni(h, count, shiftWords, stride, npx, noiseBase, segments, noiseOff, segmentCount, maxSegments);
+#endif
+    if (!pcg) build_tables();
     for (size_t i = 0; i < count; i++)
     {
       noiseBase[i] = noiseOff;
       uint32_t word;
       memcpy(&word, shiftWords + i * stride, 4);
-      const uint32_t calls = word >> 24;
-      for (uint32_t k = 0; k < calls && callCount < maxCalls; k++, noiseOff += npx[i], callCount++)
-      {
-        callState[callCount] = h; callOff[callCount] = noiseOff; callPx[callCount] = npx[i];
-        h = chain_call(h, npx[i], nullptr, false, pcg);
+      const uint32_t calls = word >> 24, n = npx[i], rounds = (!pcg && n >= 8) ? n / 8 : 0, tail = n - rounds * 8;
+      for (uint32_t k = 0; k < calls; k++, noiseOff += n)
+      {
+        uint32_t st[4];
+        const uint64_t inv = ~h;
+        memcpy(st, &h, 8);
+        memcpy(st + 2, &inv, 8);
+        uint32_t done = 0;
+        do
+        {
+          const uint32_t r = rounds - done < kNoiseSegmentRounds ? rounds - done : kNoiseSegmentRounds;
+          if (segmentCount < maxSegments)
+          {
+            NoiseSegment *seg = segments + segmentCount++;
+            memcpy(seg, st, 16);
+            seg->offset = noiseOff + 8ull * done; seg->px = 8u * r + (done + r == rounds ? tail : 0u); seg->pad = 0;
+          }
+          for (uint32_t j = 0; j < r; j++) aesdec_soft(st);
+          done += r;
+        } while (done < rounds);
+        if (rounds) memcpy(&h, st, 8);
+        for (uint32_t j = 0; j < tail; j++) (void)pcg_step(h);
       }
     }
     return h;
diff --git a/limg_amd/csrc/limg_hip_noise_gpu.hip b/limg_amd/csrc/limg_hip_noise_gpu.hip
--- a/limg_amd/csrc/limg_hip_noise_gpu.hip
+++ b/limg_amd/csrc/limg_hip_noise_gpu.hip
@@ -115,8 +115,7 @@
 
   namespace
   {
-    __global__ __launch_bounds__(256) void k_noise_expand_calls(uint8_t *noise, const unsigned long long *states, const unsigned long long *offsets, const uint32_t *pixels,
-                                                               uint32_t calls, int pcg)
+    __global__ __launch_bounds__(256) void k_noise_expand_segments(uint8_t *noise, const NoiseSegment *segments, uint32_t count, int pcg)
     {
       __shared__ uint32_t td[4][256];
       {
@@ -130,12 +129,14 @@
       }
       __syncthreads();
       const uint32_t k = blockIdx.x * 256u + threadIdx.x;
-      if (k >= calls) return;
+      if (k >= count) return;
       const uint32_t key[4] = { 0xAB705E1Du, 0x824A73EAu, 0x06CB4CADu, 0x2A76E980u };
-      unsigned long long h = states[k];
-      const uint32_t n = pixels[k], rounds = (!pcg && n >= 8u) ? n / 8u : 0u;
-      uint8_t *out = noise + offsets[k];
-      uint32_t st[4] = { (uint32_t)h, (uint32_t)(h >> 32), ~(uint32_t)h, ~(uint32_t)(h >> 32) };
+      const uint4 head = *reinterpret_cast<const uint4 *>(segments + k);
+      const uint64_t offset = segments[k].offset;
+      const uint32_t n = segments[k].px, rounds = (!pcg && n >= 8u) ? n / 8u : 0u;
+      uint8_t *out = noise + offset;
+      uint32_t st[4] = { head.x, head.y, head.z, head.w };
+      unsigned long long h = (unsigned long long)st[0] | ((unsigned long long)st[1] << 32);
       const bool aligned = (reinterpret_cast<uintptr_t>(out) & 7u) == 0;
       for (uint32_t j = 0; j < rounds; j++)
       {
@@ -163,10 +164,10 @@
     }
   }
 
-  void launch_noise_expand_calls(uint8_t *noise, const unsigned long long *dStates, const unsigned long long *dOffsets, const uint32_t *dPixels, size_t calls, bool pcg, hipStream_t s)
-  {
-    if (calls == 0) return;
-    hipLaunchKernelGGL(k_noise_expand_calls, dim3((uint32_t)((calls + 255u) / 256u)), dim3(256), 0, s, noise, dStates, dOffsets, dPixels, (uint32_t)calls, pcg ? 1 : 0);
+  void launch_noise_expand_segments(uint8_t *noise, const NoiseSegment *dSegments, size_t segments, bool pcg, hipStream_t s)
+  {
+    if (segments == 0) return;
+    hipLaunchKernelGGL(k_noise_expand_segments, dim3((uint32_t)((segments + 255u) / 256u)), dim3(256), 0, s, noise, dSegments, (uint32_t)segments, pcg ? 1 : 0);
   }
 
   void launch_noise_expand(uint8_t *noise, const unsigned long long *dStates, const uint8_t *dPixels, size_t calls, bool pcg, hipStream_t s)
```

Result: no change. 50810, median of 2 (-0.0%).
